# mrlooi/PoseCNN

Measured on AMD Instinct MI355X. Metric: frames/sec 640x480x21-class Hough-vote+RoI+ADD-loss, 1/2/4/8 MI355X, higher is better.
Workload: dtype f32 (FC GEMMs: exact 3-way split-bf16 x6 MFMA, products within 2^-24, fp32 accumulate: fp32-faithful)

## Files before the change

### include/posecnn_hip.h

```cpp
#ifndef POSECNN_HIP_H
#define POSECNN_HIP_H

#include <stddef.h>
#include <stdint.h>

#ifdef __cplusplus
extern "C" {
#endif

#define PCNN_OK 0
#define PCNN_EINVAL 1
#define PCNN_EHIP 2
#define PCNN_ECAPACITY 3

#define PCNN_MAX_ROI 128

int pcnn_abi_version(void);
const char* pcnn_strerror(int code);

int pcnn_set_completion_event(void* event);
int pcnn_completion_event_pending(void);

size_t pcnn_hough_voting_workspace_size(int B, int H, int W, int C, int skip_pixels, float vote_thr);

int pcnn_hough_voting(const int32_t* label, const float* vertex, const float* extents, const float* meta,
                      int num_meta, const float* gt, int num_gt, int B, int H, int W, int C, int batch_base,
                      int global_batch, int is_train, float inlier_thr, int label_thr, float vote_thr,
                      float per_thr, int skip_pixels, float* top_box, float* top_pose, float* top_target,
                      float* top_weight, int32_t* top_domain, int32_t* num_rois, int cap, int32_t* debug_counts,
                      void* workspace, size_t workspace_bytes, void* stream);

int pcnn_hough_voting_prob(const float* prob, int32_t* label_out, const float* vertex, const float* extents,
                           const float* meta, int num_meta, const float* gt, int num_gt, int B, int H, int W, int C,
                           int batch_base, int global_batch, int is_train, float inlier_thr, int label_thr,
                           float vote_thr, float per_thr, int skip_pixels, float* top_box, float* top_pose,
                           float* top_target, float* top_weight, int32_t* top_domain, int32_t* num_rois, int cap,
                           int32_t* debug_counts, void* workspace, size_t workspace_bytes, void* stream);

int pcnn_hough_voting_compact(const int32_t* label, const float* vertex3, const float* extents, const float* meta,
                              int num_meta, const float* gt, int num_gt, int B, int H, int W, int C, int batch_base,
                              int global_batch, int is_train, float inlier_thr, int label_thr, float vote_thr,
                              float per_thr, int skip_pixels, float* top_box, float* top_pose, float* top_target,
                              float* top_weight, int32_t* top_domain, int32_t* num_rois, int cap,
                              int32_t* debug_counts, void* workspace, size_t workspace_bytes, void* stream);

int pcnn_hough_voting_grad(float* grad_label, float* grad_vertex, int B, int H, int W, int C, void* stream);

int pcnn_hough_voting_diag(const void* workspace, int B, int H, int W, int C, int skip_pixels, float vote_thr,
                           int32_t* diag_host4, void* stream);

int pcnn_roi_pool_fwd(const float* data, int B, int H, int W, int C, int layout, const float* rois, int R_cap,
                      int roi_stride, int batch_base, const int32_t* num_rois_dev, float spatial_scale, int pooled_h, int pooled_w,
                      int pool_channel, float* top, int32_t* argmax, void* stream);

int pcnn_roi_pool_fwd_accumulate(const float* data, int B, int H, int W, int C, int layout, const float* rois,
                                 int R_cap, int roi_stride, int batch_base, const int32_t* num_rois_dev,
                                 float spatial_scale, int pooled_h, int pooled_w, int pool_channel, float* top,
                                 int32_t* argmax, void* stream);

int pcnn_roi_pool_fwd_pair(const float* data_a, int Ha, int Wa, float scale_a, const float* data_b, int Hb, int Wb,
                           float scale_b, int B, int C, const float* rois, int R_cap, int roi_stride,
                           int batch_base, const int32_t* num_rois_dev, int pooled_h, int pooled_w, float* top_sum,
                           int32_t* argmax_a, int32_t* argmax_b, void* stream);

int pcnn_roi_pool_fwd_pair_px(const float* data_a, int Ha, int Wa, float scale_a, const float* data_b, int Hb,
                              int Wb, float scale_b, int B, int C, const float* rois, int R_cap, int roi_stride,
                              int batch_base, const int32_t* num_rois_dev, int pooled_h, int pooled_w,
                              float* top_sum, uint16_t* argmax_a, uint16_t* argmax_b, void* stream);

size_t pcnn_roi_pool_bwd_workspace_size(int B, int R_cap);

int pcnn_roi_pool_bwd(const float* top_diff, const int32_t* argmax, int B, int H, int W, int C, int layout,
                      const float* rois, int R_cap, int roi_stride, int batch_base, const int32_t* num_rois_dev,
                      float spatial_scale, int pooled_h, int pooled_w, int pool_channel, float* bottom_diff,
                      void* workspace, size_t workspace_bytes, void* stream);

int pcnn_roi_pool_bwd_px(const float* top_diff, const uint16_t* argmax_px, int B, int H, int W, int C,
                         const float* rois, int R_cap, int roi_stride, int batch_base, const int32_t* num_rois_dev,
                         float spatial_scale, int pooled_h, int pooled_w, float* bottom_diff, void* workspace,
                         size_t workspace_bytes, void* stream);

size_t pcnn_add_loss_workspace_size(int R_cap, int C, int P);

int pcnn_add_loss_fwd(const float* pred, const float* target, const float* weight, const float* points,
                      const float* symmetry, int R_cap, const int32_t* num_rois_dev, int C, int P, float margin,
                      int loss_norm_rows, const int32_t* loss_norm_rows_dev, float* loss, float* bottom_diff,
                      void* workspace, size_t workspace_bytes, void* stream);

int pcnn_add_loss_prep(const float* weight, const float* symmetry, int R_cap, const int32_t* num_rois_dev, int C,
                       int P, void* workspace, size_t workspace_bytes, void* stream);
int pcnn_add_loss_fwd_prepared(const float* pred, const float* target, const float* weight, const float* points,
                               const float* symmetry, int R_cap, const int32_t* num_rois_dev, int C, int P,
                               float margin, int loss_norm_rows, const int32_t* loss_norm_rows_dev, float* loss,
                               float* bottom_diff, void* workspace, size_t workspace_bytes, void* stream);

int pcnn_add_loss_fwd_head_bwd(const float* pred, const float* target, const float* weight, const float* points,
                               const float* symmetry, int R_cap, const int32_t* num_rois_dev, int C, int P,
                               float margin, int loss_norm_rows, const int32_t* loss_norm_rows_dev,
                               float* bottom_diff, void* workspace, size_t workspace_bytes, const float* tanh_out,
                               const float* d_pred_scale, float* d_y8, void* stream);
int pcnn_add_loss_total(int R_cap, const int32_t* num_rois_dev, int C, int P, const void* workspace,
                        size_t workspace_bytes, float* loss, void* stream);

int pcnn_add_loss_bwd(const float* top_diff, const float* bottom_diff, int n, const int32_t* num_rois_dev,
                      int row_len, float* out, void* stream);

int pcnn_div_rn_check(const float* x, float b, int n, int dbl, float* out, void* stream);

int pcnn_backproject_fwd(const float* data, const float* label, const float* depth, const float* meta, int num_meta,
                         const float* label_3d, int B, int H, int W, int Ch, int NC, int grid_size,
                         int kernel_size, float threshold, float* top_data, float* top_label, float* top_flag,
                         void* stream);

int pcnn_backproject_bwd(const float* top_diff, const float* depth, const float* meta, int num_meta, int B, int H,
                         int W, int Ch, int grid_size, float* bottom_diff, void* stream);

size_t pcnn_gemm_workspace_size(int M, int N, int K, int m_dynamic, int precision);

int pcnn_gemm(int M, int N, int K, const float* A, const float* A2, int lda, int a_trans, const float* B, int ldb,
              int b_trans, float* Cm, int ldc, const float* bias, int act, const float* mask, int ldm,
              const int32_t* M_dev, const int32_t* K_dev, int precision, void* workspace, size_t workspace_bytes,
              void* stream);

int pcnn_gemm_drop(int M, int N, int K, const float* A, const float* A2, int lda, int a_trans, const float* B,
                   int ldb, int b_trans, float* Cm, int ldc, const float* bias, int act, const float* mask, int ldm,
                   const uint8_t* drop, int ldd, float keep_prob, const int32_t* M_dev, const int32_t* K_dev,
                   int precision, void* workspace, size_t workspace_bytes, void* stream);

int pcnn_gemm_drop_gen(int M, int N, int K, const float* A, const float* A2, int lda, int a_trans, const float* B,
                       int ldb, int b_trans, float* Cm, int ldc, const float* bias, int act, uint8_t* drop_out,
                       int ldd, float keep_prob, uint64_t seed, const int64_t* step_dev, int stream_id,
                       const int32_t* M_dev, const int32_t* K_dev, int precision, void* workspace,
                       size_t workspace_bytes, void* stream);

size_t pcnn_tp_bytes(int rows, int K);
int pcnn_split_tp(const float* src, long row_stride, long k_stride, int rows, const int32_t* rows_dev, int K,
                  const int32_t* K_dev, void* dst, size_t dst_bytes, void* stream);
int pcnn_gemm_tp(int M, int N, int K, const void* A_tp, const void* B_tp, float* Cm, int ldc, const float* bias,
                 int act, const float* mask, int ldm, const uint8_t* drop, int ldd, float keep_prob,
                 const int32_t* M_dev, const int32_t* K_dev, void* workspace, size_t workspace_bytes, void* stream);

int pcnn_dropout_mask(uint8_t* mask, int rows, int cols, int ld, const int32_t* rows_dev, uint64_t seed,
                      const int64_t* step_dev, int stream_id, float keep_prob, void* stream);

int pcnn_philox_check(const uint32_t* ctr, const uint32_t* key, int n, uint32_t* out, void* stream);

size_t pcnn_pose2d_workspace_size(int H, int W, int C, int n_hyp);
int pcnn_pose2d(const int32_t* label, const float* vertmap, const float* extents, int H, int W, int C, float fx,
                float fy, float px, float py, uint64_t seed, int n_hyp, int max_iter, float* poses_out,
                float* hyps_out, int32_t* hyp_px, int32_t* inl_out, int32_t* final_out, void* workspace,
                size_t workspace_bytes, void* stream);

size_t pcnn_pose3d_workspace_size(int H, int W, int C, int n_hyp);
int pcnn_pose3d(const int32_t* label, const uint16_t* depth, const float* vertmap, const float* extents, int H, int W,
                int C, float fx, float fy, float px, float py, float depth_factor, uint64_t seed, int n_hyp,
                int max_iter, int nm_evals, float* poses_out, float* hyps_out, int32_t* hyp_px, int32_t* inl_out,
                int32_t* final_out, float* energy_out, float* eye_out, void* workspace, size_t workspace_bytes,
                void* stream);

int pcnn_colsum(const float* X, int M, int N, int ldx, const int32_t* M_dev, float* out, void* stream);

int pcnn_pose_head_fwd(const float* y8, const float* poses_weight, int R_cap, const int32_t* num_rois_dev, int D,
                       float* tanh_out, float* pred, void* stream);

int pcnn_pose_head_bwd(const float* d_pred, const float* d_pred_scale, const float* tanh_out,
                       const float* poses_weight, const float* pred, int R_cap, const int32_t* num_rois_dev, int D,
                       float* d_y8, void* stream);

int pcnn_box_nms(const float* rois, int R_cap, int roi_stride, const int32_t* num_rois_dev, float thresh,
                 int32_t* keep, int32_t* num_keep, const float* poses_init, const float* poses_pred, int pred_dim,
                 float* rois_out, float* poses_out, void* stream);

int pcnn_argmax_2d(const float* prob, int B, int H, int W, int C, int32_t* label, void* stream);
int pcnn_hard_label_fwd(const float* prob, const int32_t* gt, int B, int H, int W, int C, float threshold,
                        float* top, void* stream);
int pcnn_hard_label_bwd(float* grad_prob, float* grad_gt, int B, int H, int W, int C, void* stream);

int pcnn_vertex_pred_compact(const float* feat, const float* weights, const float* bias, const int32_t* label, int B,
                             int H, int W, int K, int C, float* vertex3, void* stream);

int pcnn_icp_live_vertices(const uint16_t* depth, const int32_t* label, int H, int W, const int32_t* obj_ids, int L,
                           float factor, float fx, float fy, float px, float py, float* live, void* stream);
size_t pcnn_icp_workspace_size(int N, int H, int W);
int pcnn_icp(const float* live, int num_live, const int32_t* live_index, const float* pred_vertices,
             const float* pred_normals, int N, int H, int W, float fx, float fy, float px, float py, float znear, float zfar, float max_error,
             int iterations, const float* pose_in, float* update, float* pose_out, float* systems, void* workspace,
             size_t workspace_bytes, void* stream);
size_t pcnn_icp_reduce_workspace_size(int L, int H, int W);
int pcnn_icp_center(const float* live, const int32_t* label, const int32_t* obj_ids, int L, const float* vertmap,
                    const float* pred_vertices, const float* pred_normals, int H, int W, float max_error,
                    const float* pose_in, float* out, float* pose_out, void* workspace, size_t workspace_bytes,
                    void* stream);
size_t pcnn_energy_records_workspace_size(int N, int H, int W);
int pcnn_energy_records(const float* live, int n_live, const int32_t* label, const float* pred_vertices, int H, int W,
                        float znear, float zfar, int N, const int32_t* prob_obj, const int32_t* prob_live,
                        float* records, int32_t* counts, void* workspace, size_t workspace_bytes, void* stream);
int pcnn_energy_rec(const float* records, const int32_t* counts, int stride, const float* poses,
                    const int32_t* pose_prob, int K, float znear, float zfar, float* energy, void* stream);
int pcnn_nelder_mead_energy(const float* records, const int32_t* counts, int stride, int N, const double* x0,
                            const double* lb, const double* ub, int max_eval, float znear, float zfar, double* x_out,
                            double* f_out, int32_t* nev_out, void* stream);

size_t pcnn_nelder_mead_energy_workspace_size(int N);
int pcnn_nelder_mead_energy_coop(const float* records, const int32_t* counts, int stride, int N, const double* x0,
                                 const double* lb, const double* ub, int max_eval, float znear, float zfar,
                                 double* x_out, double* f_out, int32_t* nev_out, void* workspace,
                                 size_t workspace_bytes, void* stream);
int pcnn_nelder_mead_energy_coop_path(const float* records, const int32_t* counts, int stride, int N,
                                      const double* x0, const double* lb, const double* ub, int max_eval,
                                      float znear, float zfar, double* x_out, double* f_out, int32_t* nev_out,
                                      void* workspace, size_t workspace_bytes, int force_path, int32_t* path_out,
                                      void* stream);

size_t pcnn_icp_score_workspace_size(int J, int H, int W);
int pcnn_icp_score(const float* live, const int32_t* label, int obj, const float* vertmap, int H, int W,
                   const float* hyps, int J, float radius, float* score, int32_t* choose, void* workspace,
                   size_t workspace_bytes, void* stream);
int pcnn_pose_energy(const float* live, const int32_t* label, int obj, const float* pred_vertices, int H, int W,
                     float znear, float zfar, const float* poses, int K, float* energy, void* workspace,
                     size_t workspace_bytes, void* stream);

int pcnn_pose_energy_batch(const float* live, int n_live, const int32_t* label, const float* pred_vertices, int n_pv,
                           int H, int W, float znear, float zfar, const float* poses, int K, const int32_t* pose_obj,
                           const int32_t* pose_live, const int32_t* pose_pv, float* energy, void* workspace,
                           size_t workspace_bytes, void* stream);

size_t pcnn_render_workspace_size(int K, int H, int W, int V_total, int F_max);
int pcnn_render_meshes(const float* vertices, const float* normals, const int32_t* faces, const int32_t* vert_offset,
                       const int32_t* face_offset, int M, int V_total, int F_total, int F_max,
                       const int32_t* mesh_index, const int32_t* class_id, const float* poses, int K, int H, int W,
                       float fx, float fy, float px, float py, float znear, float zfar, float* pred_vertices,
                       float* pred_normals, float* vertmap, float* depth, int32_t* tri_id, void* workspace,
                       size_t workspace_bytes, void* stream);

#ifdef __cplusplus
}
#endif
#endif
```

### posecnn_amd/_lib.py

```python
import ctypes
import os
import threading

import torch

_HERE = os.path.dirname(os.path.abspath(__file__))
LIB_PATH = os.environ.get("POSECNN_HIP_LIB") or os.path.join(_HERE, "libposecnn_hip.so")

_lib = None
_lock = threading.Lock()

c_int = ctypes.c_int
c_float = ctypes.c_float
c_size_t = ctypes.c_size_t
c_void_p = ctypes.c_void_p

_SIGS = {
    "pcnn_abi_version": (c_int, []),
    "pcnn_strerror": (ctypes.c_char_p, [c_int]),
    "pcnn_set_completion_event": (c_int, [c_void_p]),
    "pcnn_completion_event_pending": (c_int, []),
    "pcnn_hough_voting_workspace_size": (c_size_t, [c_int, c_int, c_int, c_int, c_int, c_float]),
    "pcnn_hough_voting": (c_int, [c_void_p, c_void_p, c_void_p, c_void_p, c_int, c_void_p, c_int, c_int, c_int,
                                  c_int, c_int, c_int, c_int, c_int, c_float, c_int, c_float, c_float, c_int,
                                  c_void_p, c_void_p, c_void_p, c_void_p, c_void_p, c_void_p, c_int, c_void_p,
                                  c_void_p, c_size_t, c_void_p]),
    "pcnn_hough_voting_prob": (c_int, [c_void_p, c_void_p, c_void_p, c_void_p, c_void_p, c_int, c_void_p, c_int,
                                       c_int, c_int, c_int, c_int, c_int, c_int, c_int, c_float, c_int, c_float,
                                       c_float, c_int, c_void_p, c_void_p, c_void_p, c_void_p, c_void_p, c_void_p,
                                       c_int, c_void_p, c_void_p, c_size_t, c_void_p]),
    "pcnn_hough_voting_compact": (c_int, [c_void_p, c_void_p, c_void_p, c_void_p, c_int, c_void_p, c_int, c_int,
                                          c_int, c_int, c_int, c_int, c_int, c_int, c_float, c_int, c_float, c_float,
                                          c_int, c_void_p, c_void_p, c_void_p, c_void_p, c_void_p, c_void_p, c_int,
                                          c_void_p, c_void_p, c_size_t, c_void_p]),
    "pcnn_hough_voting_grad": (c_int, [c_void_p, c_void_p, c_int, c_int, c_int, c_int, c_void_p]),
    "pcnn_hough_voting_diag": (c_int, [c_void_p, c_int, c_int, c_int, c_int, c_int, c_float, c_void_p, c_void_p]),
    "pcnn_roi_pool_fwd": (c_int, [c_void_p, c_int, c_int, c_int, c_int, c_int, c_void_p, c_int, c_int, c_int,
                                  c_void_p, c_float, c_int, c_int, c_int, c_void_p, c_void_p, c_void_p]),
    "pcnn_roi_pool_fwd_accumulate": (c_int, [c_void_p, c_int, c_int, c_int, c_int, c_int, c_void_p, c_int, c_int,
                                             c_int, c_void_p, c_float, c_int, c_int, c_int, c_void_p, c_void_p, c_void_p]),
    "pcnn_roi_pool_fwd_pair": (c_int, [c_void_p, c_int, c_int, c_float, c_void_p, c_int, c_int, c_float, c_int, c_int,
                                       c_void_p, c_int, c_int, c_int, c_void_p, c_int, c_int, c_void_p, c_void_p,
                                       c_void_p, c_void_p]),
    "pcnn_roi_pool_fwd_pair_px": (c_int, [c_void_p, c_int, c_int, c_float, c_void_p, c_int, c_int, c_float, c_int,
                                          c_int, c_void_p, c_int, c_int, c_int, c_void_p, c_int, c_int, c_void_p,
                                          c_void_p, c_void_p, c_void_p]),
    "pcnn_roi_pool_bwd_workspace_size": (c_size_t, [c_int, c_int]),
    "pcnn_roi_pool_bwd_px": (c_int, [c_void_p, c_void_p, c_int, c_int, c_int, c_int, c_void_p, c_int, c_int, c_int,
                                     c_void_p, c_float, c_int, c_int, c_void_p, c_void_p, c_size_t, c_void_p]),
    "pcnn_roi_pool_bwd": (c_int, [c_void_p, c_void_p, c_int, c_int, c_int, c_int, c_int, c_void_p, c_int, c_int,
                                  c_int, c_void_p, c_float, c_int, c_int, c_int, c_void_p, c_void_p, c_size_t, c_void_p]),
    "pcnn_add_loss_workspace_size": (c_size_t, [c_int, c_int, c_int]),
    "pcnn_add_loss_fwd": (c_int, [c_void_p, c_void_p, c_void_p, c_void_p, c_void_p, c_int, c_void_p, c_int, c_int,
                                  c_float, c_int, c_void_p, c_void_p, c_void_p, c_void_p, c_size_t, c_void_p]),
    "pcnn_add_loss_fwd_prepared": (c_int, [c_void_p, c_void_p, c_void_p, c_void_p, c_void_p, c_int, c_void_p, c_int, c_int,
                                  c_float, c_int, c_void_p, c_void_p, c_void_p, c_void_p, c_size_t, c_void_p]),
    "pcnn_add_loss_prep": (c_int, [c_void_p, c_void_p, c_int, c_void_p, c_int, c_int, c_void_p, c_size_t, c_void_p]),
    "pcnn_add_loss_fwd_head_bwd": (c_int, [c_void_p, c_void_p, c_void_p, c_void_p, c_void_p, c_int, c_void_p, c_int,
                                           c_int, c_float, c_int, c_void_p, c_void_p, c_void_p, c_size_t, c_void_p,
                                           c_void_p, c_void_p, c_void_p]),
    "pcnn_add_loss_total": (c_int, [c_int, c_void_p, c_int, c_int, c_void_p, c_size_t, c_void_p, c_void_p]),
    "pcnn_add_loss_bwd": (c_int, [c_void_p, c_void_p, c_int, c_void_p, c_int, c_void_p, c_void_p]),
    "pcnn_div_rn_check": (c_int, [c_void_p, c_float, c_int, c_int, c_void_p, c_void_p]),
    "pcnn_backproject_fwd": (c_int, [c_void_p, c_void_p, c_void_p, c_void_p, c_int, c_void_p, c_int, c_int, c_int,
                                     c_int, c_int, c_int, c_int, c_float, c_void_p, c_void_p, c_void_p, c_void_p]),
    "pcnn_backproject_bwd": (c_int, [c_void_p, c_void_p, c_void_p, c_int, c_int, c_int, c_int, c_int, c_int,
                                     c_void_p, c_void_p]),
    "pcnn_gemm_workspace_size": (c_size_t, [c_int, c_int, c_int, c_int, c_int]),
    "pcnn_gemm": (c_int, [c_int, c_int, c_int, c_void_p, c_void_p, c_int, c_int, c_void_p, c_int, c_int, c_void_p,
                          c_int, c_void_p, c_int, c_void_p, c_int, c_void_p, c_void_p, c_int, c_void_p, c_size_t,
                          c_void_p]),
    "pcnn_gemm_drop": (c_int, [c_int, c_int, c_int, c_void_p, c_void_p, c_int, c_int, c_void_p, c_int, c_int,
                               c_void_p, c_int, c_void_p, c_int, c_void_p, c_int, c_void_p, c_int, c_float, c_void_p,
                               c_void_p, c_int, c_void_p, c_size_t, c_void_p]),
    "pcnn_gemm_drop_gen": (c_int, [c_int, c_int, c_int, c_void_p, c_void_p, c_int, c_int, c_void_p, c_int, c_int,
                                   c_void_p, c_int, c_void_p, c_int, c_void_p, c_int, c_float, ctypes.c_uint64,
                                   c_void_p, c_int, c_void_p, c_void_p, c_int, c_void_p, c_size_t, c_void_p]),
    "pcnn_dropout_mask": (c_int, [c_void_p, c_int, c_int, c_int, c_void_p, ctypes.c_uint64, c_void_p, c_int, c_float,
                                  c_void_p]),
    "pcnn_philox_check": (c_int, [c_void_p, c_void_p, c_int, c_void_p, c_void_p]),
    "pcnn_pose2d_workspace_size": (c_size_t, [c_int, c_int, c_int, c_int]),
    "pcnn_pose2d": (c_int, [c_void_p, c_void_p, c_void_p, c_int, c_int, c_int, c_float, c_float, c_float, c_float,
                            ctypes.c_uint64, c_int, c_int, c_void_p, c_void_p, c_void_p, c_void_p, c_void_p, c_void_p,
                            c_size_t, c_void_p]),
    "pcnn_pose3d_workspace_size": (c_size_t, [c_int, c_int, c_int, c_int]),
    "pcnn_pose3d": (c_int, [c_void_p, c_void_p, c_void_p, c_void_p, c_int, c_int, c_int, c_float, c_float, c_float,
                            c_float, c_float, ctypes.c_uint64, c_int, c_int, c_int, c_void_p, c_void_p, c_void_p,
                            c_void_p, c_void_p, c_void_p, c_void_p, c_void_p, c_size_t, c_void_p]),
    "pcnn_tp_bytes": (c_size_t, [c_int, c_int]),
    "pcnn_split_tp": (c_int, [c_void_p, ctypes.c_long, ctypes.c_long, c_int, c_void_p, c_int, c_void_p, c_void_p,
                              c_size_t, c_void_p]),
    "pcnn_gemm_tp": (c_int, [c_int, c_int, c_int, c_void_p, c_void_p, c_void_p, c_int, c_void_p, c_int, c_void_p,
                             c_int, c_void_p, c_int, c_float, c_void_p, c_void_p, c_void_p, c_size_t, c_void_p]),
    "pcnn_colsum": (c_int, [c_void_p, c_int, c_int, c_int, c_void_p, c_void_p, c_void_p]),
    "pcnn_box_nms": (c_int, [c_void_p, c_int, c_int, c_void_p, c_float, c_void_p, c_void_p, c_void_p, c_void_p, c_int,
                             c_void_p, c_void_p, c_void_p]),
    "pcnn_argmax_2d": (c_int, [c_void_p, c_int, c_int, c_int, c_int, c_void_p, c_void_p]),
    "pcnn_hard_label_fwd": (c_int, [c_void_p, c_void_p, c_int, c_int, c_int, c_int, c_float, c_void_p, c_void_p]),
    "pcnn_hard_label_bwd": (c_int, [c_void_p, c_void_p, c_int, c_int, c_int, c_int, c_void_p]),
    "pcnn_vertex_pred_compact": (c_int, [c_void_p, c_void_p, c_void_p, c_void_p, c_int, c_int, c_int, c_int, c_int,
                                         c_void_p, c_void_p]),
    "pcnn_pose_head_fwd": (c_int, [c_void_p, c_void_p, c_int, c_void_p, c_int, c_void_p, c_void_p, c_void_p]),
    "pcnn_pose_head_bwd": (c_int, [c_void_p, c_void_p, c_void_p, c_void_p, c_void_p, c_int, c_void_p, c_int, c_void_p,
                                   c_void_p]),
    "pcnn_icp_live_vertices": (c_int, [c_void_p, c_void_p, c_int, c_int, c_void_p, c_int, c_float, c_float, c_float,
                                       c_float, c_float, c_void_p, c_void_p]),
    "pcnn_icp_workspace_size": (c_size_t, [c_int, c_int, c_int]),
    "pcnn_icp": (c_int, [c_void_p, c_int, c_void_p, c_void_p, c_void_p, c_int, c_int, c_int, c_float, c_float, c_float,
                         c_float, c_float, c_float, c_float, c_int, c_void_p, c_void_p, c_void_p, c_void_p, c_void_p,
                         c_size_t, c_void_p]),
    "pcnn_icp_reduce_workspace_size": (c_size_t, [c_int, c_int, c_int]),
    "pcnn_icp_center": (c_int, [c_void_p, c_void_p, c_void_p, c_int, c_void_p, c_void_p, c_void_p, c_int, c_int,
                                c_float, c_void_p, c_void_p, c_void_p, c_void_p, c_size_t, c_void_p]),
    "pcnn_icp_score_workspace_size": (c_size_t, [c_int, c_int, c_int]),
    "pcnn_icp_score": (c_int, [c_void_p, c_void_p, c_int, c_void_p, c_int, c_int, c_void_p, c_int, c_float, c_void_p,
                               c_void_p, c_void_p, c_size_t, c_void_p]),
    "pcnn_energy_records_workspace_size": (c_size_t, [c_int, c_int, c_int]),
    "pcnn_energy_records": (c_int, [c_void_p, c_int, c_void_p, c_void_p, c_int, c_int, c_float, c_float, c_int,
                                    c_void_p, c_void_p, c_void_p, c_void_p, c_void_p, c_size_t, c_void_p]),
    "pcnn_energy_rec": (c_int, [c_void_p, c_void_p, c_int, c_void_p, c_void_p, c_int, c_float, c_float, c_void_p,
                                c_void_p]),
    "pcnn_nelder_mead_energy": (c_int, [c_void_p, c_void_p, c_int, c_int, c_void_p, c_void_p, c_void_p, c_int,
                                        c_float, c_float, c_void_p, c_void_p, c_void_p, c_void_p]),
    "pcnn_nelder_mead_energy_workspace_size": (c_size_t, [c_int]),
    "pcnn_nelder_mead_energy_coop": (c_int, [c_void_p, c_void_p, c_int, c_int, c_void_p, c_void_p, c_void_p, c_int,
                                             c_float, c_float, c_void_p, c_void_p, c_void_p, c_void_p, c_size_t,
                                             c_void_p]),
    "pcnn_nelder_mead_energy_coop_path": (c_int, [c_void_p, c_void_p, c_int, c_int, c_void_p, c_void_p, c_void_p,
                                                  c_int, c_float, c_float, c_void_p, c_void_p, c_void_p, c_void_p,
                                                  c_size_t, c_int, c_void_p, c_void_p]),
    "pcnn_pose_energy_batch": (c_int, [c_void_p, c_int, c_void_p, c_void_p, c_int, c_int, c_int, c_float, c_float,
                                       c_void_p, c_int, c_void_p, c_void_p, c_void_p, c_void_p, c_void_p, c_size_t,
                                       c_void_p]),
    "pcnn_pose_energy": (c_int, [c_void_p, c_void_p, c_int, c_void_p, c_int, c_int, c_float, c_float, c_void_p, c_int,
                                 c_void_p, c_void_p, c_size_t, c_void_p]),
    "pcnn_render_workspace_size": (c_size_t, [c_int, c_int, c_int, c_int, c_int]),
    "pcnn_render_meshes": (c_int, [c_void_p, c_void_p, c_void_p, c_void_p, c_void_p, c_int, c_int, c_int, c_int,
                                   c_void_p, c_void_p, c_void_p, c_int, c_int, c_int, c_float, c_float, c_float,
                                   c_float, c_float, c_float, c_void_p, c_void_p, c_void_p, c_void_p, c_void_p,
                                   c_void_p, c_size_t, c_void_p]),
}


class PcnnError(RuntimeError):
    pass


def load():
    global _lib
    if _lib is not None:
        return _lib
    with _lock:
        if _lib is None:
            if not os.path.exists(LIB_PATH):
                raise PcnnError(f"{LIB_PATH} not built; run __graft_entry__.build() "
                                "(hipcc --offload-arch=gfx950). No CPU fallback exists.")
            lib = ctypes.CDLL(LIB_PATH)
            for name, (res, args) in _SIGS.items():
                if name.endswith("_check") and not hasattr(lib, name):
                    continue
                fn = getattr(lib, name)
                fn.restype = res
                fn.argtypes = args
            _lib = lib
    return _lib


def exported_symbols():
    return list(_SIGS.keys())


def check(rc, what):
    if rc != 0:
        msg = load().pcnn_strerror(rc).decode()
        if rc == 1:
            raise ValueError(f"{what}: {msg}")
        raise PcnnError(f"{what}: {msg} (code {rc})")


def require_gpu(*tensors):
    if not torch.cuda.is_available():
        raise PcnnError("posecnn_amd ops run only on an AMD GPU (HIP); none is visible")
    for t in tensors:
        if t is not None and not t.is_cuda:
            raise ValueError("posecnn_amd ops take device tensors (got a CPU tensor)")


def ptr(t):
    return None if t is None else ctypes.c_void_p(t.data_ptr())


def stream_ptr(stream=None):
    s = stream if stream is not None else torch.cuda.current_stream()
    return ctypes.c_void_p(s.cuda_stream)


_ws = {}


def workspace(nbytes, device, tag="default", stream=None):
    s = stream if stream is not None else torch.cuda.current_stream(device)
    key = (str(device), tag, s.cuda_stream)
    buf = _ws.get(key)
    if buf is None or buf.numel() < nbytes:
        with torch.cuda.stream(s):
            buf = torch.empty(max(int(nbytes), 256), dtype=torch.uint8, device=device)
        _ws[key] = buf
    return buf
```

### posecnn_amd/csrc/roi_pooling.hip

```cpp
#include "pcnn_common.h"
#include <math.h>
#include <cfloat>

namespace {


struct RoiGeo {
  int b, cls, sw, sh, ew, eh;
  float bin_h, bin_w;
};

__device__ __forceinline__ RoiGeo roi_geo(const float* __restrict__ rois, int r, int stride, int batch_base,
                                          float scale, int PH, int PW) {
  const float* o = rois + (size_t)r * stride;
  RoiGeo g;
  g.b = (int)o[0] - batch_base;
  const int c0 = stride == 5 ? 1 : 2;
  g.cls = stride == 5 ? 0 : (int)o[1];
  g.sw = (int)roundf(o[c0 + 0] * scale);
  g.sh = (int)roundf(o[c0 + 1] * scale);
  g.ew = (int)roundf(o[c0 + 2] * scale);
  g.eh = (int)roundf(o[c0 + 3] * scale);
  const int roi_w = max(g.ew - g.sw + 1, 1);
  const int roi_h = max(g.eh - g.sh + 1, 1);
  g.bin_h = (float)roi_h / (float)PH;
  g.bin_w = (float)roi_w / (float)PW;
  return g;
}

__device__ __forceinline__ int rows_of(const int32_t* num_rois_dev, int R_cap) {
  if (!num_rois_dev) return R_cap;
  int r = *num_rois_dev;
  return r < R_cap ? r : R_cap;
}

__device__ __forceinline__ void bin_bounds(const RoiGeo& g, int ph, int pw, int H, int W, int& hs, int& he, int& ws,
                                           int& we) {
  hs = (int)floorf((float)ph * g.bin_h);
  ws = (int)floorf((float)pw * g.bin_w);
  he = (int)ceilf((float)(ph + 1) * g.bin_h);
  we = (int)ceilf((float)(pw + 1) * g.bin_w);
  hs = min(max(hs + g.sh, 0), H);
  he = min(max(he + g.sh, 0), H);
  ws = min(max(ws + g.sw, 0), W);
  we = min(max(we + g.sw, 0), W);
}

__device__ __forceinline__ void bins_of_pixel(const RoiGeo& g, int h, int w, int PH, int PW, int& phs, int& phe,
                                              int& pws, int& pwe) {
  phs = (int)floorf((float)(h - g.sh) / g.bin_h);
  phe = (int)ceilf((float)(h - g.sh + 1) / g.bin_h);
  pws = (int)floorf((float)(w - g.sw) / g.bin_w);
  pwe = (int)ceilf((float)(w - g.sw + 1) / g.bin_w);
  phs = min(max(phs, 0), PH);
  phe = min(max(phe, 0), PH);
  pws = min(max(pws, 0), PW);
  pwe = min(max(pwe, 0), PW);
}

__device__ __forceinline__ void upd(float v, int idx, float& m, int& a) {
  if (v > m) { m = v; a = idx; }
}

constexpr int kXcds = 8;
constexpr int kRun = 9;
__device__ __forceinline__ bool fwd_item(int R, int nbins, int& r, int& bin) {
  const int id = blockIdx.x;
  const int x = id % kXcds, local = id / kXcds;
  const int lr = local / nbins;
  bin = local % nbins;
  r = ((lr / kRun) * kXcds + x) * kRun + lr % kRun;
  return r < R;
}
static inline unsigned fwd_grid(int R_cap, int nbins) {
  return (unsigned)(kXcds * ((R_cap + kXcds * kRun - 1) / (kXcds * kRun)) * kRun * nbins);
}

template <bool PX = false>
__device__ __forceinline__ void bin_max4(const float* __restrict__ data, int B, int H, int W, int C,
                                         const RoiGeo& g, int ph, int pw, int c, float4& m, int4& a) {
  const bool bad = g.b < 0 || g.b >= B;
  int hs, he, ws, we;
  bin_bounds(g, ph, pw, H, W, hs, he, ws, we);
  const bool empty = bad || (he <= hs) || (we <= ws);
  const float* bd = data + (size_t)(bad ? 0 : g.b) * H * W * C;
  float m0, m1, m2, m3;
  m0 = m1 = m2 = m3 = empty ? 0.f : -FLT_MAX;
  int a0 = -1, a1 = -1, a2 = -1, a3 = -1;
  if (!empty) {
    for (int h = hs; h < he; h++) {
      int w = ws;
      for (; w + 1 < we; w += 2) {
        const int i0 = (h * W + w) * C + c, i1 = i0 + C;
        const float4 v0 = *(const float4*)(bd + i0);
        const float4 v1 = *(const float4*)(bd + i1);
        if (PX) {
          const int p0 = h * W + w, p1 = p0 + 1;
          upd(v0.x, p0, m0, a0); upd(v0.y, p0, m1, a1); upd(v0.z, p0, m2, a2); upd(v0.w, p0, m3, a3);
          upd(v1.x, p1, m0, a0); upd(v1.y, p1, m1, a1); upd(v1.z, p1, m2, a2); upd(v1.w, p1, m3, a3);
        } else {
          upd(v0.x, i0 + 0, m0, a0); upd(v0.y, i0 + 1, m1, a1); upd(v0.z, i0 + 2, m2, a2); upd(v0.w, i0 + 3, m3, a3);
          upd(v1.x, i1 + 0, m0, a0); upd(v1.y, i1 + 1, m1, a1); upd(v1.z, i1 + 2, m2, a2); upd(v1.w, i1 + 3, m3, a3);
        }
      }
      if (w < we) {
        const int i0 = (h * W + w) * C + c;
        const float4 v0 = *(const float4*)(bd + i0);
        if (PX) {
          const int p0 = h * W + w;
          upd(v0.x, p0, m0, a0); upd(v0.y, p0, m1, a1); upd(v0.z, p0, m2, a2); upd(v0.w, p0, m3, a3);
        } else {
          upd(v0.x, i0 + 0, m0, a0); upd(v0.y, i0 + 1, m1, a1); upd(v0.z, i0 + 2, m2, a2); upd(v0.w, i0 + 3, m3, a3);
        }
      }
    }
  }
  m = make_float4(m0, m1, m2, m3);
  a = make_int4(a0, a1, a2, a3);
}

template <bool ACC>
__global__ void __launch_bounds__(128) k_roi_fwd_nhwc4(const float* __restrict__ data, int B, int H, int W, int C,
                                                        const float* __restrict__ rois, int R_cap, int stride,
                                                        int batch_base, const int32_t* __restrict__ num_rois_dev,
                                                        float scale, int PH, int PW, float* __restrict__ top,
                                                        int32_t* __restrict__ argmax) {
  int r, bin;
  if (!fwd_item(rows_of(num_rois_dev, R_cap), PH * PW, r, bin)) return;
  const int ph = bin / PW, pw = bin % PW;
  const RoiGeo g = roi_geo(rois, r, stride, batch_base, scale, PH, PW);
  float* to = top + (((size_t)r * PH + ph) * PW + pw) * C;
  int32_t* ao = argmax + (((size_t)r * PH + ph) * PW + pw) * C;
  for (int c = threadIdx.x * 4; c < C; c += blockDim.x * 4) {
    float4 m;
    int4 a;
    bin_max4(data, B, H, W, C, g, ph, pw, c, m, a);
    if (ACC) {
      const float4 p = *(const float4*)(to + c);
      *(float4*)(to + c) = make_float4(p.x + m.x, p.y + m.y, p.z + m.z, p.w + m.w);
    } else {
      *(float4*)(to + c) = m;
    }
    *(int4*)(ao + c) = a;
  }
}

template <bool PX>
__global__ void __launch_bounds__(128) k_roi_fwd_pair_nhwc4(const float* __restrict__ data_a, int Ha, int Wa,
                                                             float scale_a, const float* __restrict__ data_b, int Hb,
                                                             int Wb, float scale_b, int B, int C,
                                                             const float* __restrict__ rois, int R_cap, int stride,
                                                             int batch_base, const int32_t* __restrict__ num_rois_dev,
                                                             int PH, int PW, float* __restrict__ top,
                                                             void* __restrict__ arg_a, void* __restrict__ arg_b) {
  int r, bin;
  if (!fwd_item(rows_of(num_rois_dev, R_cap), PH * PW, r, bin)) return;
  const int ph = bin / PW, pw = bin % PW;
  const RoiGeo ga = roi_geo(rois, r, stride, batch_base, scale_a, PH, PW);
  const RoiGeo gb = roi_geo(rois, r, stride, batch_base, scale_b, PH, PW);
  const size_t o = (((size_t)r * PH + ph) * PW + pw) * C;
  for (int c = threadIdx.x * 4; c < C; c += blockDim.x * 4) {
    float4 ma, mb;
    int4 aa, ab;
    bin_max4<PX>(data_a, B, Ha, Wa, C, ga, ph, pw, c, ma, aa);
    bin_max4<PX>(data_b, B, Hb, Wb, C, gb, ph, pw, c, mb, ab);
    *(float4*)(top + o + c) = make_float4(ma.x + mb.x, ma.y + mb.y, ma.z + mb.z, ma.w + mb.w);
    if (PX) {
      auto pk = [](int4 a) {
        return make_uint2(((unsigned)a.x & 0xFFFFu) | ((unsigned)a.y << 16),
                          ((unsigned)a.z & 0xFFFFu) | ((unsigned)a.w << 16));
      };
      *(uint2*)((uint16_t*)arg_a + o + c) = pk(aa);
      *(uint2*)((uint16_t*)arg_b + o + c) = pk(ab);
    } else {
      *(int4*)((int32_t*)arg_a + o + c) = aa;
      *(int4*)((int32_t*)arg_b + o + c) = ab;
    }
  }
}

__global__ void k_roi_fwd_generic(const float* __restrict__ data, int B, int H, int W, int C, int layout,
                                  const float* __restrict__ rois, int R_cap, int stride, int batch_base,
                                  const int32_t* __restrict__ num_rois_dev, float scale, int PH, int PW,
                                  int pool_channel, int acc, float* __restrict__ top, int32_t* __restrict__ argmax) {
  const int R = rows_of(num_rois_dev, R_cap);
  const int Co = pool_channel ? 1 : C;
  const long n_out = (long)R * PH * PW * Co;
  for (long idx = (long)blockIdx.x * blockDim.x + threadIdx.x; idx < n_out; idx += (long)gridDim.x * blockDim.x) {
    int r, ph, pw, c;
    if (layout == 0) {
      long t = idx;
      c = (int)(t % Co); t /= Co;
      pw = (int)(t % PW); t /= PW;
      ph = (int)(t % PH); r = (int)(t / PH);
    } else {
      long t = idx;
      pw = (int)(t % PW); t /= PW;
      ph = (int)(t % PH); t /= PH;
      c = (int)(t % Co); r = (int)(t / Co);
    }
    const RoiGeo g = roi_geo(rois, r, stride, batch_base, scale, PH, PW);
    const bool bad = g.b < 0 || g.b >= B;
    const int ch = pool_channel ? g.cls : c;
    int hs, he, ws, we;
    bin_bounds(g, ph, pw, H, W, hs, he, ws, we);
    const bool empty = bad || (he <= hs) || (we <= ws) || ch < 0 || ch >= C;
    float maxval = empty ? 0.f : -FLT_MAX;
    int maxidx = -1;
    if (!empty) {
      const float* bd = data + (size_t)g.b * H * W * C;
      for (int h = hs; h < he; h++)
        for (int w = ws; w < we; w++) {
          const int bi = layout == 0 ? (h * W + w) * C + ch : (ch * H + h) * W + w;
          const float v = bd[bi];
          if (v > maxval) { maxval = v; maxidx = bi; }
        }
    }
    top[idx] = acc ? top[idx] + maxval : maxval;
    argmax[idx] = maxidx;
  }
}

__global__ void __launch_bounds__(1024) k_roi_prep(const float* __restrict__ rois, int R_cap, int stride,
                                                    int batch_base, const int32_t* __restrict__ num_rois_dev, int B,
                                                    float scale, int PH, int PW, int32_t* __restrict__ geo,
                                                    int32_t* __restrict__ lo, int32_t* __restrict__ hi) {
  __shared__ int slo[1024], shi[1024];
  const int R = rows_of(num_rois_dev, R_cap);
  const int nb = B < 1024 ? B : 1024;
  for (int b = threadIdx.x; b < nb; b += blockDim.x) {
    slo[b] = 0x7fffffff;
    shi[b] = -1;
  }
  __syncthreads();
  for (int r = threadIdx.x; r < R; r += blockDim.x) {
    const RoiGeo g = roi_geo(rois, r, stride, batch_base, scale, PH, PW);
    int32_t* o = geo + (size_t)r * 8;
    o[0] = g.b; o[1] = g.cls; o[2] = g.sw; o[3] = g.sh; o[4] = g.ew; o[5] = g.eh;
    o[6] = __float_as_int(g.bin_h);
    o[7] = __float_as_int(g.bin_w);
    if (g.b >= 0 && g.b < nb) {
      atomicMin(&slo[g.b], r);
      atomicMax(&shi[g.b], r);
    }
  }
  __syncthreads();
  for (int b = threadIdx.x; b < B; b += blockDim.x) {
    lo[b] = b < nb ? slo[b] : 0;
    hi[b] = b < nb ? shi[b] : -1;
  }
}

#ifndef PCNN_RBW_NARROW
#define PCNN_RBW_NARROW 8192
#endif
constexpr int kBWaves = 1;
constexpr int kBChunk = 128 * kBWaves;
constexpr int kBGroup = 16;
constexpr int kBCap = kBGroup * 49;
constexpr int kBBatch = 8;

template <int kBTH, int kBTW, bool PX>
__global__ void __launch_bounds__(64 * kBWaves) k_roi_bwd_ent(const float* __restrict__ top_diff,
                                                               const void* __restrict__ argmax, int B, int H, int W,
                                                               int C, const int32_t* __restrict__ geo,
                                                               const int32_t* __restrict__ lo,
                                                               const int32_t* __restrict__ hi, int PH, int PW,
                                                               float* __restrict__ bottom) {
  constexpr int kBPix = kBTH * kBTW;
  __shared__ int2 ent[kBCap];
  __shared__ int sh_total;
  const int tiles_w = (W + kBTW - 1) / kBTW, tiles_h = (H + kBTH - 1) / kBTH;
  const int nchunk = (C + kBChunk - 1) / kBChunk;
  const int ipx = (int)((gridDim.x + 7) / 8);
  int id = (int)(blockIdx.x % 8) * ipx + (int)(blockIdx.x / 8);
  if (id >= B * tiles_w * tiles_h * nchunk) return;
  const int chunk = id % nchunk;
  id /= nchunk;
  const int t = id % (tiles_w * tiles_h), b = id / (tiles_w * tiles_h);
  const int h0 = (t / tiles_w) * kBTH, w0 = (t % tiles_w) * kBTW;
  const int th = min(kBTH, H - h0), tw = min(kBTW, W - w0);
  const int lane = pcnn::lane_id(), wave = threadIdx.x >> 6;
  const int c = chunk * kBChunk + 2 * threadIdx.x;
  const bool cok = c < C;
  float2 acc[kBPix];
  int expv[kBPix];
#pragma unroll
  for (int p = 0; p < kBPix; p++) {
    acc[p] = make_float2(0.f, 0.f);
    const int pix = (h0 + p / kBTW) * W + w0 + p % kBTW;
    expv[p] = PX ? pix : pix * C + c;
  }
  constexpr int kNext = PX ? 0 : 1;
  const int r0 = lo[b], r1 = hi[b];
  const __amdgpu_buffer_rsrc_t rs_t = __builtin_amdgcn_make_buffer_rsrc((void*)top_diff, (short)0, 0x7fffffff, 0x00020000);
  const __amdgpu_buffer_rsrc_t rs_a = __builtin_amdgcn_make_buffer_rsrc((void*)argmax, (short)0, 0x7fffffff, 0x00020000);
  const unsigned voff = cok ? (unsigned)c * 4u : 0x80000000u;
  const unsigned voff_a = cok ? (unsigned)c * (PX ? 2u : 4u) : 0x80000000u;
  for (int rb = r0; rb <= r1; rb += 64) {
    uint32_t rbits = 0;
    uint32_t cbits = 0;
    const int r = rb + lane;
    if (wave == 0 && r <= r1) {
      const int32_t* gg = geo + (size_t)r * 8;
      RoiGeo g;
      g.b = gg[0]; g.sw = gg[2]; g.sh = gg[3]; g.ew = gg[4]; g.eh = gg[5];
      g.bin_h = __int_as_float(gg[6]);
      g.bin_w = __int_as_float(gg[7]);
      if (g.b == b && g.sh <= h0 + th - 1 && g.eh >= h0 && g.sw <= w0 + tw - 1 && g.ew >= w0) {
        for (int i = 0; i < th; i++) {
          const int h = h0 + i;
          if (h < g.sh || h > g.eh) continue;
          int s0 = (int)floorf((float)(h - g.sh) / g.bin_h), e0 = (int)ceilf((float)(h - g.sh + 1) / g.bin_h);
          s0 = min(max(s0, 0), PH);
          e0 = min(max(e0, 0), PH);
          for (int ph = s0; ph < e0; ph++) rbits |= 1u << (ph * kBTH + i);
        }
        for (int j = 0; j < tw; j++) {
          const int w = w0 + j;
          if (w < g.sw || w > g.ew) continue;
          int s0 = (int)floorf((float)(w - g.sw) / g.bin_w), e0 = (int)ceilf((float)(w - g.sw + 1) / g.bin_w);
          s0 = min(max(s0, 0), PW);
          e0 = min(max(e0, 0), PW);
          for (int pw = s0; pw < e0; pw++) cbits |= 1u << (pw * kBTW + j);
        }
      }
    }
    const uint64_t hits = __ballot(rbits && cbits);
    for (int g0 = 0; g0 < 64; g0 += kBGroup) {
      if (wave == 0) {
        const uint64_t gm = hits & (((1ull << kBGroup) - 1) << g0);
        const bool mine = (gm >> lane) & 1;
        int cnt = 0;
        if (mine) {
          int nph = 0, npw = 0;
          for (int ph = 0; ph < PH; ph++) nph += ((rbits >> (ph * kBTH)) & ((1u << kBTH) - 1)) != 0;
          for (int pw = 0; pw < PW; pw++) npw += ((cbits >> (pw * kBTW)) & ((1u << kBTW) - 1)) != 0;
          cnt = nph * npw;
        }
        int off = cnt;
#pragma unroll
        for (int d = 1; d < 64; d <<= 1) {
          const int v = __shfl_up(off, d, 64);
          if (lane >= d) off += v;
        }
        if (lane == 63) sh_total = off;
        off -= cnt;
        if (mine) {
          const int rbase = r * PH;
          for (int ph = 0; ph < PH; ph++) {
            const uint32_t rm = (rbits >> (ph * kBTH)) & ((1u << kBTH) - 1);
            if (!rm) continue;
            for (int pw = 0; pw < PW; pw++) {
              const uint32_t cm = (cbits >> (pw * kBTW)) & ((1u << kBTW) - 1);
              if (!cm) continue;
              uint32_t m = 0;
#pragma unroll
              for (int i = 0; i < kBTH; i++)
                if ((rm >> i) & 1) m |= cm << (i * kBTW);
              ent[off++] = make_int2(((rbase + ph) * PW + pw) * C, (int)m);
            }
          }
        }
      }
      __syncthreads();
      const int total = sh_total;
      auto fetch = [&](int e0, int2& my, int2 (&av)[kBBatch], float2 (&dv)[kBBatch]) {
        my = ent[min(e0 + (lane & (kBBatch - 1)), total - 1)];
#pragma unroll
        for (int k = 0; k < kBBatch; k++) {
          const int so = __builtin_amdgcn_readlane(my.x, k) * 4;
          if (PX) {
            const unsigned a2 = __builtin_amdgcn_raw_buffer_load_b32(rs_a, voff_a, so >> 1, 0);
            av[k] = make_int2((int)(a2 & 0xFFFFu), (int)(a2 >> 16));
          } else {
            av[k] = __builtin_bit_cast(int2, __builtin_amdgcn_raw_buffer_load_b64(rs_a, voff_a, so, 0));
          }
          dv[k] = __builtin_bit_cast(float2, __builtin_amdgcn_raw_buffer_load_b64(rs_t, voff, so, 0));
        }
      };
      auto accumulate = [&](int e0, const int2& my, const int2 (&av)[kBBatch], const float2 (&dv)[kBBatch]) {
#pragma unroll
        for (int k = 0; k < kBBatch; k++) {
          if (e0 + k >= total) break;
          const uint32_t m = (uint32_t)__builtin_amdgcn_readlane(my.y, k);
#pragma unroll
          for (int q = 0; q < kBPix; q++) {
            if (!((m >> q) & 1)) continue;
            acc[q].x += av[k].x == expv[q] ? dv[k].x : 0.f;
            acc[q].y += av[k].y == expv[q] + kNext ? dv[k].y : 0.f;
          }
        }
      };
      if (total > 0) {
        int2 myA, myB, avA[kBBatch], avB[kBBatch];
        float2 dvA[kBBatch], dvB[kBBatch];
        fetch(0, myA, avA, dvA);
        for (int e0 = 0; e0 < total; e0 += 2 * kBBatch) {
          if (e0 + kBBatch < total) fetch(e0 + kBBatch, myB, avB, dvB);
          accumulate(e0, myA, avA, dvA);
          if (e0 + 2 * kBBatch < total) fetch(e0 + 2 * kBBatch, myA, avA, dvA);
          if (e0 + kBBatch < total) accumulate(e0 + kBBatch, myB, avB, dvB);
        }
      }
      __syncthreads();
    }
  }
  if (cok) {
#pragma unroll
    for (int i = 0; i < kBTH; i++)
#pragma unroll
      for (int j = 0; j < kBTW; j++)
        if (i < th && j < tw) *(float2*)(bottom + (((size_t)b * H + h0 + i) * W + w0 + j) * C + c) = acc[i * kBTW + j];
  }
}

__global__ void k_roi_bwd_generic(const float* __restrict__ top_diff, const int32_t* __restrict__ argmax, int B,
                                  int H, int W, int C, int layout, const int32_t* __restrict__ geo, int PH, int PW,
                                  int pool_channel, const int32_t* __restrict__ lo, const int32_t* __restrict__ hi,
                                  float* __restrict__ bottom) {
  const long npix = (long)B * H * W;
  const int Co = pool_channel ? 1 : C;
  for (long pi = (long)blockIdx.x * blockDim.x + threadIdx.x; pi < npix; pi += (long)gridDim.x * blockDim.x) {
    const int w = (int)(pi % W), h = (int)((pi / W) % H), b = (int)(pi / ((long)W * H));
    const int r0 = lo[b], r1 = hi[b];
    for (int r = r0; r <= r1; r++) {
      const int32_t* gg = geo + (size_t)r * 8;
      RoiGeo g;
      g.b = gg[0]; g.cls = gg[1]; g.sw = gg[2]; g.sh = gg[3]; g.ew = gg[4]; g.eh = gg[5];
      g.bin_h = __int_as_float(gg[6]);
      g.bin_w = __int_as_float(gg[7]);
      if (g.b != b) continue;
      if (!(w >= g.sw && w <= g.ew && h >= g.sh && h <= g.eh)) continue;
      int phs, phe, pws, pwe;
      bins_of_pixel(g, h, w, PH, PW, phs, phe, pws, pwe);
      const int cb = pool_channel ? g.cls : 0, ce = pool_channel ? g.cls + 1 : C;
      if (cb < 0 || ce > C) continue;
      for (int c = cb; c < ce; c++) {
        const int bidx = layout == 0 ? (h * W + w) * C + c : (c * H + h) * W + w;
        float* dst = bottom + (size_t)b * H * W * C + bidx;
        float acc = *dst;
        for (int ph = phs; ph < phe; ph++)
          for (int pw = pws; pw < pwe; pw++) {
            const int oc = pool_channel ? 0 : c;
            const size_t t = layout == 0 ? (((size_t)r * PH + ph) * PW + pw) * Co + oc
                                         : (((size_t)r * Co + oc) * PH + ph) * PW + pw;
            if (argmax[t] == bidx) acc += top_diff[t];
          }
        *dst = acc;
      }
    }
  }
}

}

static int roi_pool_fwd(const float* data, int B, int H, int W, int C, int layout, const float* rois, int R_cap,
                        int roi_stride, int batch_base, const int32_t* num_rois_dev, float spatial_scale,
                        int pooled_h, int pooled_w, int pool_channel, int acc, float* top, int32_t* argmax,
                        void* stream) {
  PCNN_REQUIRE(data && rois && top && argmax && B > 0 && H > 0 && W > 0 && C > 0 && R_cap >= 0);
  PCNN_REQUIRE(pooled_h > 0 && pooled_w > 0 && (layout == 0 || layout == 1));
  PCNN_REQUIRE(roi_stride >= 6 || (roi_stride == 5 && !pool_channel));
  PCNN_REQUIRE((long)H * W * C < (1l << 31));
  if (R_cap == 0) return PCNN_OK;
  hipStream_t st = (hipStream_t)stream;
  const bool vec = layout == 0 && !pool_channel && C % 4 == 0 && (((uintptr_t)data | (uintptr_t)top |
                                                                    (uintptr_t)argmax) & 15) == 0;
  if (vec) {
    const int threads = C / 4 >= 128 ? 128 : ((C / 4 + 63) / 64) * 64;
    if (acc)
      hipLaunchKernelGGL(k_roi_fwd_nhwc4<true>, dim3(fwd_grid(R_cap, pooled_h * pooled_w)), dim3(threads), 0, st, data, B, H,
                         W, C, rois, R_cap, roi_stride, batch_base, num_rois_dev, spatial_scale, pooled_h, pooled_w, top,
                         argmax);
    else
      hipLaunchKernelGGL(k_roi_fwd_nhwc4<false>, dim3(fwd_grid(R_cap, pooled_h * pooled_w)), dim3(threads), 0, st, data, B, H,
                         W, C, rois, R_cap, roi_stride, batch_base, num_rois_dev, spatial_scale, pooled_h, pooled_w, top,
                         argmax);
  } else {
    const long n = (long)R_cap * pooled_h * pooled_w * (pool_channel ? 1 : C);
    const int blocks = (int)((n + 255) / 256 < 8192 ? (n + 255) / 256 : 8192);
    hipLaunchKernelGGL(k_roi_fwd_generic, dim3(blocks), dim3(256), 0, st, data, B, H, W, C, layout, rois, R_cap,
                       roi_stride, batch_base, num_rois_dev, spatial_scale, pooled_h, pooled_w, pool_channel, acc, top,
                       argmax);
  }
  PCNN_CHECK_LAUNCH();
  return PCNN_OK;
}

extern "C" int pcnn_roi_pool_fwd(const float* data, int B, int H, int W, int C, int layout, const float* rois,
                                 int R_cap, int roi_stride, int batch_base, const int32_t* num_rois_dev,
                                 float spatial_scale, int pooled_h, int pooled_w, int pool_channel, float* top,
                                 int32_t* argmax, void* stream) {
  return roi_pool_fwd(data, B, H, W, C, layout, rois, R_cap, roi_stride, batch_base, num_rois_dev, spatial_scale,
                      pooled_h,
                      pooled_w, pool_channel, 0, top, argmax, stream);
}

extern "C" int pcnn_roi_pool_fwd_accumulate(const float* data, int B, int H, int W, int C, int layout,
                                            const float* rois, int R_cap, int roi_stride, int batch_base,
                                            const int32_t* num_rois_dev, float spatial_scale, int pooled_h,
                                            int pooled_w, int pool_channel, float* top, int32_t* argmax,
                                            void* stream) {
  return roi_pool_fwd(data, B, H, W, C, layout, rois, R_cap, roi_stride, batch_base, num_rois_dev, spatial_scale,
                      pooled_h,
                      pooled_w, pool_channel, 1, top, argmax, stream);
}

static int roi_pool_fwd_pair(const float* data_a, int Ha, int Wa, float scale_a, const float* data_b, int Hb, int Wb,
                             float scale_b, int B, int C, const float* rois, int R_cap, int roi_stride, int batch_base,
                             const int32_t* num_rois_dev, int pooled_h, int pooled_w, float* top_sum, void* argmax_a,
                             void* argmax_b, bool px, void* stream) {
  PCNN_REQUIRE(data_a && data_b && rois && top_sum && argmax_a && argmax_b && B > 0 && C > 0 && C % 4 == 0);
  PCNN_REQUIRE(Ha > 0 && Wa > 0 && Hb > 0 && Wb > 0 && pooled_h > 0 && pooled_w > 0 && R_cap >= 0);
  PCNN_REQUIRE(roi_stride >= 5);
  PCNN_REQUIRE((long)Ha * Wa * C < (1l << 31) && (long)Hb * Wb * C < (1l << 31));
  PCNN_REQUIRE(!px || ((long)Ha * Wa < 0xFFFF && (long)Hb * Wb < 0xFFFF));
  PCNN_REQUIRE(((((uintptr_t)data_a) | ((uintptr_t)data_b) | ((uintptr_t)top_sum)) & 15) == 0);
  PCNN_REQUIRE(((((uintptr_t)argmax_a) | ((uintptr_t)argmax_b)) & (px ? 7 : 15)) == 0);
  if (R_cap == 0) return PCNN_OK;
  const int threads = C / 4 >= 128 ? 128 : ((C / 4 + 63) / 64) * 64;
  if (px)
    hipLaunchKernelGGL(k_roi_fwd_pair_nhwc4<true>, dim3(fwd_grid(R_cap, pooled_h * pooled_w)), dim3(threads), 0,
                       (hipStream_t)stream, data_a, Ha, Wa, scale_a, data_b, Hb, Wb, scale_b, B, C, rois, R_cap,
                       roi_stride, batch_base, num_rois_dev, pooled_h, pooled_w, top_sum, argmax_a, argmax_b);
  else
    hipLaunchKernelGGL(k_roi_fwd_pair_nhwc4<false>, dim3(fwd_grid(R_cap, pooled_h * pooled_w)), dim3(threads), 0,
                       (hipStream_t)stream, data_a, Ha, Wa, scale_a, data_b, Hb, Wb, scale_b, B, C, rois, R_cap,
                       roi_stride, batch_base, num_rois_dev, pooled_h, pooled_w, top_sum, argmax_a, argmax_b);
  PCNN_CHECK_LAUNCH();
  return PCNN_OK;
}

extern "C" int pcnn_roi_pool_fwd_pair(const float* data_a, int Ha, int Wa, float scale_a, const float* data_b, int Hb,
                                      int Wb, float scale_b, int B, int C, const float* rois, int R_cap, int roi_stride,
                                      int batch_base, const int32_t* num_rois_dev, int pooled_h, int pooled_w, float* top_sum,
                                      int32_t* argmax_a, int32_t* argmax_b, void* stream) {
  return roi_pool_fwd_pair(data_a, Ha, Wa, scale_a, data_b, Hb, Wb, scale_b, B, C, rois, R_cap, roi_stride, batch_base,
                           num_rois_dev, pooled_h, pooled_w, top_sum, argmax_a, argmax_b, false, stream);
}

extern "C" int pcnn_roi_pool_fwd_pair_px(const float* data_a, int Ha, int Wa, float scale_a, const float* data_b,
                                         int Hb, int Wb, float scale_b, int B, int C, const float* rois, int R_cap,
                                         int roi_stride, int batch_base, const int32_t* num_rois_dev, int pooled_h,
                                         int pooled_w, float* top_sum, uint16_t* argmax_a, uint16_t* argmax_b,
                                         void* stream) {
  return roi_pool_fwd_pair(data_a, Ha, Wa, scale_a, data_b, Hb, Wb, scale_b, B, C, rois, R_cap, roi_stride, batch_base,
                           num_rois_dev, pooled_h, pooled_w, top_sum, argmax_a, argmax_b, true, stream);
}

extern "C" size_t pcnn_roi_pool_bwd_workspace_size(int B, int R_cap) {
  return pcnn::align_up((size_t)2 * (B > 0 ? B : 1) * sizeof(int32_t), 256) +
         pcnn::align_up((size_t)(R_cap > 0 ? R_cap : 1) * 8 * sizeof(int32_t), 256) + 256;
}

static int roi_pool_bwd(const float* top_diff, const void* argmax, bool px, int B, int H, int W, int C, int layout,
                        const float* rois, int R_cap, int roi_stride, int batch_base, const int32_t* num_rois_dev,
                        float spatial_scale, int pooled_h, int pooled_w, int pool_channel, float* bottom_diff,
                        void* workspace, size_t workspace_bytes, void* stream) {
  PCNN_REQUIRE(top_diff && argmax && rois && bottom_diff && workspace && B > 0 && H > 0 && W > 0 && C > 0);
  PCNN_REQUIRE(pooled_h > 0 && pooled_w > 0 && (layout == 0 || layout == 1) && R_cap >= 0);
  PCNN_REQUIRE(roi_stride >= 6 || (roi_stride == 5 && !pool_channel));
  PCNN_REQUIRE((long)H * W * C < (1l << 31));
  if (workspace_bytes < pcnn_roi_pool_bwd_workspace_size(B, R_cap)) return PCNN_ECAPACITY;
  hipStream_t st = (hipStream_t)stream;
  pcnn::Carve cv(workspace);
  int32_t* lo = cv.take<int32_t>(B);
  int32_t* hi = cv.take<int32_t>(B);
  int32_t* geo = cv.take<int32_t>((size_t)(R_cap > 0 ? R_cap : 1) * 8);
  hipLaunchKernelGGL(k_roi_prep, dim3(1), dim3(1024), 0, st, rois, R_cap, roi_stride, batch_base, num_rois_dev,
                     B, spatial_scale, pooled_h, pooled_w, geo, lo, hi);
  const int nchunk = (C + kBChunk - 1) / kBChunk;
  const long wg24 = (long)B * ((H + 1) / 2) * ((W + 3) / 4) * nchunk;
  const bool narrow = wg24 < PCNN_RBW_NARROW;
#ifndef PCNN_RBW_TH
#define PCNN_RBW_TH 2
#endif
  const int tbh = narrow ? 1 : PCNN_RBW_TH, tbw = 4;
  const bool vec = layout == 0 && !pool_channel && C % 2 == 0 && pooled_h * tbh <= 32 && pooled_w * tbw <= 32 &&
                   (long)H * W * C < (1l << 30) && (long)R_cap * pooled_h * pooled_w * C < (1l << 29) &&
                   (((uintptr_t)top_diff | (uintptr_t)bottom_diff) & 7) == 0 && ((uintptr_t)argmax & (px ? 3 : 7)) == 0;
  PCNN_REQUIRE(!px || (vec && (long)H * W < 0xFFFF));
  if (vec) {
    const int tiles = ((H + tbh - 1) / tbh) * ((W + tbw - 1) / tbw);
    const unsigned nwg = (unsigned)((B * tiles * nchunk + 7) / 8 * 8);
#define PCNN_RBW(TH, PXV)                                                                                  \
  pcnn::launch_last(k_roi_bwd_ent<TH, 4, PXV>, dim3(nwg), dim3(64 * kBWaves), 0, st, top_diff, argmax, B, H, W, C, \
                    geo, lo, hi, pooled_h, pooled_w, bottom_diff)
    if (narrow) {
      if (px) PCNN_RBW(1, true); else PCNN_RBW(1, false);
    } else {
      if (px) PCNN_RBW(PCNN_RBW_TH, true); else PCNN_RBW(PCNN_RBW_TH, false);
    }
#undef PCNN_RBW
  } else {
    if (hipMemsetAsync(bottom_diff, 0, (size_t)B * H * W * C * sizeof(float), st) != hipSuccess) return PCNN_EHIP;
    const long npix = (long)B * H * W;
    const int blocks = (int)((npix + 255) / 256 < 8192 ? (npix + 255) / 256 : 8192);
    hipLaunchKernelGGL(k_roi_bwd_generic, dim3(blocks), dim3(256), 0, st, top_diff, (const int32_t*)argmax, B, H, W,
                       C, layout, geo, pooled_h, pooled_w, pool_channel, lo, hi, bottom_diff);
  }
  PCNN_CHECK_LAUNCH();
  return PCNN_OK;
}

extern "C" int pcnn_roi_pool_bwd(const float* top_diff, const int32_t* argmax, int B, int H, int W, int C, int layout,
                                 const float* rois, int R_cap, int roi_stride, int batch_base,
                                 const int32_t* num_rois_dev, float spatial_scale, int pooled_h, int pooled_w,
                                 int pool_channel, float* bottom_diff, void* workspace, size_t workspace_bytes, void* stream) {
  return roi_pool_bwd(top_diff, argmax, false, B, H, W, C, layout, rois, R_cap, roi_stride, batch_base, num_rois_dev,
                      spatial_scale, pooled_h, pooled_w, pool_channel, bottom_diff, workspace, workspace_bytes, stream);
}

extern "C" int pcnn_roi_pool_bwd_px(const float* top_diff, const uint16_t* argmax_px, int B, int H, int W, int C,
                                    const float* rois, int R_cap, int roi_stride, int batch_base,
                                    const int32_t* num_rois_dev, float spatial_scale, int pooled_h, int pooled_w,
                                    float* bottom_diff, void* workspace, size_t workspace_bytes, void* stream) {
  return roi_pool_bwd(top_diff, argmax_px, true, B, H, W, C, 0, rois, R_cap, roi_stride, batch_base, num_rois_dev,
                      spatial_scale, pooled_h, pooled_w, 0, bottom_diff, workspace, workspace_bytes, stream);
}
```

### posecnn_amd/pipeline.py

```python
import contextlib

import torch

from . import _lib
from . import pose_head as ph
from .hough_voting_gpu_layer import hough_voting_gpu_op as hv
from .roi_pooling_layer import roi_pooling_op as rp
from .average_distance_loss import average_distance_loss_op as adl
from .exchange import GradShard, RoiExchange

CAP = hv.CAPACITY
_nullctx = contextlib.nullcontext


class PoseStep:
    def __init__(self, B, H, W, num_classes, device, conv4_hw=None, conv5_hw=None, channels=512, units=4096,
                 is_train=1, skip_pixels=10, vote_threshold=-1.0, vote_percentage=0.02, margin=0.01,
                 global_batch=None, batch_base=0, weights=None, dist=None, backward=True, precision=2,
                 overlap_weight_grads=True, pixel_argmax=True, keep_prob=None, drop_seed=0x5EED, side_prep=True,
                 drop_in_reduce=True, pipeline=False, prefetch_at="loss", fuse_loss_tail=True,
                 defer_side_join=False, signal_forks=True, pool_at_tail=False):
        self.B, self.H, self.W, self.C = B, H, W, num_classes
        self.dev = device
        self.is_train, self.skip, self.vthr, self.vper, self.margin = is_train, skip_pixels, vote_threshold, \
            vote_percentage, margin
        self.global_batch = global_batch or B
        self.batch_base = batch_base
        self.dist = dist
        self.backward = backward
        self.prec = precision
        self.h4, self.w4 = conv4_hw or (H // 8, W // 8)
        self.h5, self.w5 = conv5_hw or (H // 16, W // 16)
        self.Ch = channels
        D = 4 * num_classes
        self.D = D
        self.weights = weights or ph.PoseHeadWeights(num_classes, device, in_dim=49 * channels, units=units)
        f32 = dict(dtype=torch.float32, device=device)
        i32 = dict(dtype=torch.int32, device=device)
        K6 = 49 * channels
        px = pixel_argmax and max(self.h4 * self.w4, self.h5 * self.w5) < 0xFFFF
        adt = dict(dtype=torch.int16 if px else torch.int32, device=device)

        def minibatch_set():
            return dict(hough=dict(box=torch.zeros((CAP, 7), **f32), pose=torch.zeros((CAP, 7), **f32),
                                   target=torch.zeros((CAP, D), **f32), weight=torch.zeros((CAP, D), **f32),
                                   domain=torch.zeros((CAP,), **i32), num_rois=torch.zeros((2,), **i32)),
                        pool=torch.zeros((CAP, 7, 7, channels), **f32),
                        arg5=torch.zeros((CAP, 7, 7, channels), **adt),
                        arg4=torch.zeros((CAP, 7, 7, channels), **adt),
                        add_ws=None, prepped=False)
        self.fuse_loss_tail = fuse_loss_tail
        self.pipeline = bool(pipeline)
        self._sets = [minibatch_set() for _ in range(2 if self.pipeline else 1)]
        self._cur = 0
        self._primed = None
        self.prefetch_at = prefetch_at
        if prefetch_at not in ("loss", "bwd", "start", "fwd", "tail"):
            raise ValueError("prefetch_at must be 'start', 'fwd', 'loss', 'bwd' or 'tail'")
        self._fork_ev = torch.cuda.Event() if self.pipeline else None
        self._fork_recorded = False
        self.pre_stream = torch.cuda.Stream(device=device) if self.pipeline else None
        self._next = None
        self.y6 = torch.zeros((CAP, units), **f32)
        self.y7 = torch.zeros((CAP, units), **f32)
        self.y8 = torch.zeros((CAP, D), **f32)
        self.t8 = torch.zeros((CAP, D), **f32)
        self.pred = torch.zeros((CAP, D), **f32)
        self.loss = torch.zeros((1,), **f32)
        self.diff = torch.zeros((CAP, D), **f32)
        self.one = torch.ones((1,), **f32)
        self.dy8 = torch.zeros((CAP, D), **f32)
        self.dy7 = torch.zeros((CAP, units), **f32)
        self.dy6 = torch.zeros((CAP, units), **f32)
        self.dx = torch.zeros((CAP, K6), **f32)
        self.gshard = None
        if dist is not None:
            per_max = 9 if is_train else 1
            slot = max(1, min(CAP, B * (hv.MAX_ROI // self.global_batch) * per_max))
            self.gshard = GradShard(dist, slot, [("w6", (K6, units)), ("w7", (units, units)), ("w8", (units, D))],
                                    device)
        self.grads = self.weights.grads_like()
        if self.gshard is not None:
            for k in ("w6", "w7", "w8"):
                self.grads[k] = self.grads[k][self.gshard.rows(k)].contiguous()
        self.keep = float(keep_prob if keep_prob is not None else (0.5 if is_train else 1.0))
        if not 0.0 < self.keep <= 1.0:
            raise ValueError("keep_prob must be in (0, 1]")
        self.drop6 = self.drop7 = None
        self._drop_external = False
        self.drop_in_reduce = drop_in_reduce
        self._bump_drop_step = False
        self._drawn = False
        if self.keep < 1.0:
            u8 = dict(dtype=torch.uint8, device=device)
            self.drop6 = torch.zeros((CAP, units), **u8)
            self.drop7 = torch.zeros((CAP, units), **u8)
            self.drop_step = torch.zeros((1,), dtype=torch.int64, device=device)
            rank = dist.get_rank() if dist is not None else 0
            self.drop_seed = (int(drop_seed) + rank * 0x9E3779B97F4A7C15) & ((1 << 64) - 1)
            self._drop_ready = None
            self._drop_ev = torch.cuda.Event()
        self.dconv4 = torch.zeros((B, self.h4, self.w4, channels), **f32)
        self.dconv5 = torch.zeros((B, self.h5, self.w5, channels), **f32)
        self.norm_rows = torch.zeros((1,), **i32)
        self.timer = None
        self.gemm_timer = None
        self.xchg = None
        self.detections = None
        self._pending = {}
        self._in_step = False
        self.side_stream = torch.cuda.Stream(device=device) if overlap_weight_grads else None
        self.side_prep = side_prep and self.side_stream is not None
        self.defer_side_join = bool(defer_side_join) and self.pipeline and dist is None and \
            self.side_stream is not None
        self._side_mid_ev = torch.cuda.Event() if self.defer_side_join else None
        self._side_done_ev = torch.cuda.Event() if self.defer_side_join else None
        self._side_pending = False
        self.signal_forks = bool(signal_forks) and self.side_stream is not None and dist is None
        self._fork_evs = {}
        self.pool_at_tail = bool(pool_at_tail) and self.pipeline
        self._pool_pending = None
        if self.signal_forks:
            for k in ("loss", "fc8_dx", "fc7_dx"):
                ev = torch.cuda.Event()
                ev.record()
                self._fork_evs[k] = ev
        self._mid_covers_pre = False
        self._mid_waited = False

    def _t(self, name):
        step = self

        class _Ctx:
            def __enter__(self_):
                if step.timer is not None:
                    self_.e0 = torch.cuda.Event(enable_timing=True)
                    self_.e0.record()

            def __exit__(self_, *a):
                if step.timer is not None:
                    e1 = torch.cuda.Event(enable_timing=True)
                    e1.record()
                    step.timer.setdefault(name, []).append((self_.e0, e1))
        return _Ctx()

    def join(self):
        cur = torch.cuda.current_stream()
        for st in (self.side_stream, self.pre_stream):
            if st is not None:
                cur.wait_stream(st)
        self._side_pending = False

    def _side_wait(self, ev_name, stream=None):
        if self._side_pending:
            (stream or torch.cuda.current_stream()).wait_event(getattr(self, ev_name))

    def _arm_fork(self, name):
        if not self.signal_forks or self.timer is not None or torch.cuda.is_current_stream_capturing():
            return None
        ev = self._fork_evs[name]
        _lib.load().pcnn_set_completion_event(ev.cuda_event)
        return ev

    @staticmethod
    def _fork_taken(ev):
        if ev is None:
            return None
        return None if _lib.load().pcnn_completion_event_pending() else ev

    def _fork_side(self, side, ev):
        if ev is not None:
            side.wait_event(ev)
        else:
            side.wait_stream(torch.cuda.current_stream())

    hough = property(lambda self: self._sets[self._cur]["hough"])
    pool = property(lambda self: self._sets[self._cur]["pool"])
    arg5 = property(lambda self: self._sets[self._cur]["arg5"])
    arg4 = property(lambda self: self._sets[self._cur]["arg4"])
    add_ws = property(lambda self: self._sets[self._cur]["add_ws"])

    def vote(self, label, vertex, extents, meta, gt, s=None):
        s = self._cur if s is None else s
        self._sets[s]["pooled"] = False
        with self._t("hough_voting_gpu"):
            return hv.hough_voting_gpu_capacity(label, vertex, extents, meta, gt, self.is_train, self.vthr,
                                                self.vper, self.skip, global_batch=self.global_batch,
                                                batch_base=self.batch_base, out=self._sets[s]["hough"])

    def add_prep(self, points, symmetry, s=None, stream=None):
        s = self._cur if s is None else s
        st = self._sets[s]
        if st["add_ws"] is None:
            st["add_ws"] = torch.empty(adl.workspace_bytes(CAP, self.C, points.shape[1]), dtype=torch.uint8,
                                       device=self.dev)
        h = st["hough"]
        side = None
        if stream is None:
            side = self.side_stream if self.timer is None and self.side_prep else None
            if side is not None:
                side.wait_stream(torch.cuda.current_stream())
        with torch.cuda.stream(stream or side or torch.cuda.current_stream()):
            adl.average_distance_loss_prep(h["weight"], symmetry, points.shape[1], st["add_ws"],
                                           num_rois=h["num_rois"][1:2])
        st["prepped"] = "side" if side is not None else "stream"

    def pool_fwd(self, conv4, conv5, s=None):
        s = self._cur if s is None else s
        st = self._sets[s]
        with self._t("roi_pool_fwd"):
            rp.roi_pool_pair(conv5, 1.0 / 16.0, conv4, 1.0 / 8.0, st["hough"]["box"], 7, 7,
                             num_rois=st["hough"]["num_rois"][1:2], out=(st["pool"], st["arg5"], st["arg4"]),
                             batch_base=self.batch_base)
        st["pooled"] = True

    def _front(self, inputs, s, stream=None):
        ctx = torch.cuda.stream(stream) if stream is not None else _nullctx()
        with ctx:
            self.vote(inputs["label"], inputs["vertex"], inputs["extents"], inputs["meta"], inputs["gt"], s=s)
            if stream is not None:
                self.add_prep(inputs["points"], inputs["symmetry"], s=s, stream=stream)
                if self.pool_at_tail and stream is self.pre_stream:
                    self._pool_pending = (inputs, s)
                else:
                    self.pool_fwd(inputs["conv4"], inputs["conv5"], s=s)

    def _issue_pending_pool(self):
        if self._pool_pending is None:
            return
        inputs, s = self._pool_pending
        self._pool_pending = None
        with torch.cuda.stream(self.pre_stream):
            self.pool_fwd(inputs["conv4"], inputs["conv5"], s=s)

    def _prefetch(self):
        if self._next is None:
            return
        nxt, s = self._next
        self._next = None
        if self.timer is not None:
            self._side_wait("_side_done_ev")
            self._side_pending = False
            self._front(nxt, s, stream=torch.cuda.current_stream())
        else:
            if self._fork_recorded:
                self.pre_stream.wait_event(self._fork_ev)
            else:
                self.pre_stream.wait_stream(torch.cuda.current_stream())
            self._side_wait("_side_done_ev", self.pre_stream)
            self._front(nxt, s, stream=self.pre_stream)
        self._fork_recorded = False
        self._primed = (s, nxt)

    def set_drop_masks(self, m6, m7):
        if self.keep >= 1.0:
            raise ValueError("set_drop_masks: the step has keep_prob 1 (no dropout)")
        for dst, m in ((self.drop6, m6), (self.drop7, m7)):
            dst.zero_()
            dst[:m.shape[0]].copy_(m.to(torch.uint8))
        self._drop_external = True

    def draw_drop_masks(self):
        if self.keep >= 1.0 or self._drop_external or self.drop_in_reduce:
            return
        self._drawn = True
        nr = self.hough["num_rois"][1:2]
        side = self.side_stream if self.timer is None and self.side_prep else None
        if side is not None:
            side.wait_stream(torch.cuda.current_stream())
        with torch.cuda.stream(side or torch.cuda.current_stream()):
            ph.dropout_mask(self.drop6, self.keep, self.drop_seed, self.drop_step, 6, rows_dev=nr)
            ph.dropout_mask(self.drop7, self.keep, self.drop_seed, self.drop_step, 7, rows_dev=nr)
            self.drop_step.add_(1)
            if side is not None:
                self._drop_ev.record(side)
                self._drop_ready = self._drop_ev

    def exchange(self):
        h = self.hough
        if self.dist is None:
            self.norm_rows = h["num_rois"][1:2]
            return
        with self._t("allreduce_rows"):
            self.norm_rows.copy_(h["num_rois"][0:1])
            self._pending["rows"] = self.dist.all_reduce(self.norm_rows, async_op=True)

    def _wait(self, key):
        w = self._pending.pop(key, None)
        if w is not None:
            w.wait()

    def gather_detections(self):
        h = self.hough
        if self.dist is None:
            return torch.cat([h["box"], h["pose"]], 1), h["num_rois"][0:1]
        return self._exchange_rows()(h["box"], h["pose"], h["num_rois"])

    def _exchange_rows(self):
        if self.xchg is None:
            self.xchg = RoiExchange(self.dist, CAP, self.dev)
        return self.xchg

    def forward(self, conv4, conv5, points, symmetry):
        h = self.hough
        nr = h["num_rois"][1:2]
        w = self.weights
        K6 = 49 * self.Ch
        st = self._sets[self._cur]
        if not (self.pipeline and st.get("pooled")):
            self.pool_fwd(conv4, conv5)
        x = self.pool.view(CAP, K6)
        gs = self.gshard if self.backward else None
        if gs is not None:
            gs.send_input("w6", x)
        dk = dict(keep_prob=self.keep) if self.keep < 1.0 else {}
        if not self._drawn:
            self.draw_drop_masks()
        self._drawn = False
        if self.keep < 1.0 and getattr(self, "_drop_ready", None) is not None:
            torch.cuda.current_stream().wait_event(self._drop_ready)
            self._drop_ready = None
        gen = self.keep < 1.0 and self.drop_in_reduce and not self._drop_external
        g6 = dict(drop_gen=(self.drop_seed, self.drop_step, 6)) if gen else {}
        g7 = dict(drop_gen=(self.drop_seed, self.drop_step, 7)) if gen else {}
        if not self._mid_waited:
            self._side_wait("_side_mid_ev")
        self._mid_waited = False
        with self._t("gemm_fc6_fwd"):
            self._g("fc6_fwd", x, w.w6, self.y6, bias=w.b6, act=1, M_dev=nr, drop=self.drop6, **dk, **g6)
        if self.prefetch_at == "fwd":
            self._prefetch()
        if gs is not None:
            gs.send_input("w7", self.y6)
        with self._t("gemm_fc7_fc8_fwd"):
            self._g("fc7_fwd", self.y6, w.w7, self.y7, bias=w.b7, act=1, M_dev=nr, drop=self.drop7, **dk, **g7)
            if gs is not None:
                gs.send_input("w8", self.y7)
            self._g("fc8_fwd", self.y7, w.w8, self.y8, bias=w.b8, act=0, M_dev=nr)
        if self.prefetch_at == "loss":
            self._prefetch()
        if gen:
            if self._in_step and self.backward:
                self._bump_drop_step = True
            else:
                self.drop_step.add_(1)
        if self.dist is not None:
            self._wait("rows")
            self.norm_rows.clamp_(min=1)
        with self._t("head_add_loss_fwd"):
            ph.head_fwd(self.y8, h["weight"], self.t8, self.pred, num_rois=nr)
            if not st["prepped"]:
                self.add_prep(points, symmetry)
            if st["prepped"] == "side":
                torch.cuda.current_stream().wait_stream(self.side_stream)
            st["prepped"] = False
            self._wait("loss")
            side = self.side_stream
            self._head_bwd_done = fuse = (self.fuse_loss_tail and self._in_step and self.backward and
                                          self.timer is None and side is not None and self.D <= 256)
            if fuse:
                ev = self._arm_fork("loss")
                adl.average_distance_loss_head_bwd(self.pred, h["target"], h["weight"], points, symmetry,
                                                   self.margin, self.t8, self.one, self.diff, self.dy8, st["add_ws"],
                                                   num_rois=nr, loss_norm_rows_dev=self.norm_rows)
                self._fork_side(side, self._fork_taken(ev))
                with torch.cuda.stream(side):
                    adl.average_distance_loss_total(CAP, self.C, points.shape[1], st["add_ws"], self.loss,
                                                    num_rois=nr)
                    if self.dist is not None:
                        self._pending["loss"] = self.dist.all_reduce(self.loss, async_op=True)
                return self.loss
            adl.average_distance_loss(self.pred, h["target"], h["weight"], points, symmetry, self.margin,
                                      num_rois=nr, loss_norm_rows_dev=self.norm_rows, out=(self.loss, self.diff),
                                      workspace=st["add_ws"], prepared=True)
        if self.dist is not None:
            self._pending["loss"] = self.dist.all_reduce(self.loss, async_op=True)
            if not self._in_step:
                self._wait("loss")
        return self.loss

    def backward_pass(self, conv4, conv5):
        h = self.hough
        nr = h["num_rois"][1:2]
        w, g = self.weights, self.grads
        K6 = 49 * self.Ch
        main = torch.cuda.current_stream()
        side = self.side_stream if self.timer is None else None
        gs = self.gshard
        x = self.pool.view(CAP, K6)

        def weight_grads(name, X, dY, K_loc, M, N, fork=True, fork_ev=None):
            if side is not None and fork:
                self._fork_side(side, fork_ev)
            if gs is not None:
                gs.send_grad(name, dY, nr)
            with torch.cuda.stream(side or main):
                if gs is not None:
                    gs.reduce(name, g[name], g["b" + name[1:]],
                              lambda A, B_, C_, **kw: self._g(f"fc{name[1:]}_dw", A, B_, C_, **kw), ph.colsum)
                else:
                    ph.colsum(dY, g["b" + name[1:]], M_dev=nr)
                    self._g(f"fc{name[1:]}_dw", X, dY, g[name], a_trans=1, K_dev=nr, M=M, N=N, K=K_loc)

        fused_fork = getattr(self, "_head_bwd_done", False) and side is not None
        if not getattr(self, "_head_bwd_done", False):
            with self._t("add_loss_head_bwd"):
                ph.head_bwd(self.diff, self.t8, h["weight"], self.pred, self.dy8, num_rois=nr,
                            d_pred_scale=self.one)
        self._head_bwd_done = False
        if self.prefetch_at == "bwd":
            self._prefetch()
        with self._t("gemm_fc8_fc7_dw_bias"):
            weight_grads("w8", self.y7, self.dy8, CAP, w.units, self.D, fork=not fused_fork)
        dk = dict(keep_prob=self.keep) if self.keep < 1.0 else {}
        ev = self._arm_fork("fc8_dx") if side is not None else None
        with self._t("gemm_fc8_fc7_dx"):
            self._g("fc8_dx", self.dy8, w.w8, self.dy7, b_trans=1, mask=self.y7, M_dev=nr, **dk)
        ev = self._fork_taken(ev)
        with self._t("gemm_fc8_fc7_dw_bias"):
            weight_grads("w7", self.y6, self.dy7, CAP, w.units, w.units, fork_ev=ev)
        defer = self.defer_side_join and side is not None
        self._side_wait("_side_done_ev")
        self._side_pending = False
        if defer:
            self._mid_covers_pre = (self._primed is not None and self._pool_pending is None and
                                    not torch.cuda.is_current_stream_capturing())
            if self._mid_covers_pre:
                side.wait_stream(self.pre_stream)
            if self._bump_drop_step and self._mid_covers_pre:
                with torch.cuda.stream(side):
                    self.drop_step.add_(1)
                self._bump_drop_step = False
            self._side_mid_ev.record(side)
        ev = self._arm_fork("fc7_dx") if side is not None else None
        with self._t("gemm_fc8_fc7_dx"):
            self._g("fc7_dx", self.dy7, w.w7, self.dy6, b_trans=1, mask=self.y6, M_dev=nr, **dk)
        ev = self._fork_taken(ev)
        with self._t("gemm_fc6_dw"):
            weight_grads("w6", x, self.dy6, CAP, K6, w.units, fork_ev=ev)
        with self._t("gemm_fc6_dx"):
            self._g("fc6_dx", self.dy6, w.w6, self.dx, b_trans=1, M_dev=nr)
        if self.prefetch_at == "tail":
            self._prefetch()
        self._issue_pending_pool()
        dxp = self.dx.view(CAP, 7, 7, self.Ch)
        with self._t("roi_pool_bwd"):
            rp.roi_pool_grad(conv5, h["box"], self.arg5, dxp, 7, 7, 1.0 / 16.0, 0, num_rois=nr, out=self.dconv5,
                             batch_base=self.batch_base)
            rp.roi_pool_grad(conv4, h["box"], self.arg4, dxp, 7, 7, 1.0 / 8.0, 0, num_rois=nr, out=self.dconv4,
                             batch_base=self.batch_base)
        if self._bump_drop_step:
            self.drop_step.add_(1)
            self._bump_drop_step = False
        if defer:
            self._side_done_ev.record(side)
            self._side_pending = True
        elif side is not None:
            main.wait_stream(side)

    def _g(self, name, A, B, C, **kw):
        if self.gemm_timer is None:
            return ph.gemm(A, B, C, precision=self.prec, **kw)
        e0, e1 = torch.cuda.Event(enable_timing=True), torch.cuda.Event(enable_timing=True)
        e0.record()
        ph.gemm(A, B, C, precision=self.prec, **kw)
        e1.record()
        self.gemm_timer.setdefault(name, []).append((e0, e1))
        return C

    def step(self, inputs, next_inputs=None):
        if self.pipeline:
            return self._step_pipelined(inputs, next_inputs)
        if next_inputs is not None:
            raise ValueError("next_inputs needs PoseStep(pipeline=True)")
        self.vote(inputs["label"], inputs["vertex"], inputs["extents"], inputs["meta"], inputs["gt"])
        self.draw_drop_masks()
        if self.side_prep:
            self.add_prep(inputs["points"], inputs["symmetry"])
        return self._train(inputs)

    def _step_pipelined(self, inputs, next_inputs):
        main = torch.cuda.current_stream()
        if self._primed is not None and self._primed[1] is inputs:
            self._cur = self._primed[0]
            if self._side_pending and self._mid_covers_pre:
                main.wait_event(self._side_mid_ev)
                self._mid_waited = True
            else:
                main.wait_stream(self.pre_stream)
        else:
            self._side_wait("_side_done_ev")
            self._side_pending = False
            self._front(inputs, self._cur, stream=main)
        self._primed = None
        self._next = (next_inputs, 1 - self._cur) if next_inputs is not None else None
        self.draw_drop_masks()
        if self.prefetch_at == "start":
            self._prefetch()
        elif self.prefetch_at == "fwd" and self._next is not None and self.timer is None:
            self._fork_ev.record(main)
            self._fork_recorded = True
        loss = self._train(inputs)
        self._prefetch()
        self._issue_pending_pool()
        return loss

    def _train(self, inputs):
        self.exchange()
        if self.dist is not None:
            with self._t("allgather_rois"):
                h = self.hough
                self._exchange_rows().start(h["box"], h["pose"], h["num_rois"])
        self._in_step = True
        try:
            loss = self.forward(inputs["conv4"], inputs["conv5"], inputs["points"], inputs["symmetry"])
            if self.backward:
                self.backward_pass(inputs["conv4"], inputs["conv5"])
        finally:
            self._in_step = False
        self._wait("loss")
        if self.dist is not None:
            rows, total = self.xchg.finish()
            self.detections = (rows.clone(), total.clone())
        return loss
```

### posecnn_amd/roi_pooling_layer/roi_pooling_op.py

```python
import torch

from .. import _lib


def roi_pool(bottom_data, bottom_rois, pooled_height, pooled_width, spatial_scale, pool_channel=0, name=None,
             num_rois=None, layout=0, out=None, accumulate=False, batch_base=0):
    _lib.require_gpu(bottom_data, bottom_rois)
    if bottom_data.dim() != 4:
        raise ValueError("data must be 4-dimensional")
    if bottom_rois.dim() != 2:
        raise ValueError("rois must be 2-dimensional")
    data = bottom_data.contiguous().float()
    rois = bottom_rois.contiguous().float()
    if layout == 0:
        B, H, W, C = data.shape
    else:
        B, C, H, W = data.shape
    R, stride = rois.shape
    Co = 1 if pool_channel else C
    shape = (R, pooled_height, pooled_width, Co) if layout == 0 else (R, Co, pooled_height, pooled_width)
    if out is None:
        if accumulate:
            raise ValueError("accumulate=True needs out=(top, argmax)")
        top = torch.empty(shape, dtype=torch.float32, device=data.device)
        arg = torch.empty(shape, dtype=torch.int32, device=data.device)
    else:
        top, arg = out
    lib = _lib.load()
    fn = lib.pcnn_roi_pool_fwd_accumulate if accumulate else lib.pcnn_roi_pool_fwd
    rc = fn(_lib.ptr(data), B, H, W, C, layout, _lib.ptr(rois), R, stride, int(batch_base), _lib.ptr(num_rois),
            float(spatial_scale), int(pooled_height), int(pooled_width), int(pool_channel), _lib.ptr(top),
            _lib.ptr(arg), _lib.stream_ptr())
    _lib.check(rc, "roi_pool")
    return top, arg


def roi_pool_pair(data_a, scale_a, data_b, scale_b, rois, pooled_height, pooled_width, num_rois=None, out=None,
                  batch_base=0, pixel_argmax=False):
    _lib.require_gpu(data_a, data_b, rois)
    if data_a.dim() != 4 or data_b.dim() != 4 or rois.dim() != 2:
        raise ValueError("data must be 4-dimensional and rois 2-dimensional")
    da, db = data_a.contiguous().float(), data_b.contiguous().float()
    B, Ha, Wa, C = da.shape
    Bb, Hb, Wb, Cb = db.shape
    if (Bb, Cb) != (B, C):
        raise ValueError("both maps need the same batch and channel count")
    rois = rois.contiguous().float()
    R, stride = rois.shape
    shape = (R, pooled_height, pooled_width, C)
    if out is None:
        adt = torch.int16 if pixel_argmax else torch.int32
        out = (torch.empty(shape, dtype=torch.float32, device=da.device),
               torch.empty(shape, dtype=adt, device=da.device),
               torch.empty(shape, dtype=adt, device=da.device))
    top, arg_a, arg_b = out
    if arg_a.dtype != arg_b.dtype or arg_a.dtype not in (torch.int16, torch.int32):
        raise ValueError("argmax tensors must both be int32 (flat index) or int16 (pixel index)")
    fn = _lib.load().pcnn_roi_pool_fwd_pair_px if arg_a.dtype == torch.int16 else _lib.load().pcnn_roi_pool_fwd_pair
    rc = fn(_lib.ptr(da), Ha, Wa, float(scale_a), _lib.ptr(db), Hb, Wb, float(scale_b), B, C, _lib.ptr(rois), R, stride,
            int(batch_base), _lib.ptr(num_rois), int(pooled_height), int(pooled_width), _lib.ptr(top), _lib.ptr(arg_a),
            _lib.ptr(arg_b), _lib.stream_ptr())
    _lib.check(rc, "roi_pool_pair")
    return top, arg_a, arg_b


def roi_pool_grad(bottom_data, bottom_rois, argmax, grad, pooled_height, pooled_width, spatial_scale,
                  pool_channel=0, name=None, num_rois=None, layout=0, out=None, batch_base=0):
    _lib.require_gpu(bottom_data, bottom_rois, argmax, grad)
    rois = bottom_rois.contiguous().float()
    if layout == 0:
        B, H, W, C = bottom_data.shape
    else:
        B, C, H, W = bottom_data.shape
    R, stride = rois.shape
    lib = _lib.load()
    ws = _lib.workspace(lib.pcnn_roi_pool_bwd_workspace_size(B, R), bottom_data.device, "roi_bwd")
    dd = out if out is not None else torch.empty(bottom_data.shape, dtype=torch.float32, device=bottom_data.device)
    if argmax.dtype == torch.int16:
        if layout != 0 or pool_channel:
            raise ValueError("a pixel-index argmax needs NHWC data and pool_channel 0")
        rc = lib.pcnn_roi_pool_bwd_px(_lib.ptr(grad.contiguous()), _lib.ptr(argmax.contiguous()), B, H, W, C,
                                      _lib.ptr(rois), R, stride, int(batch_base), _lib.ptr(num_rois),
                                      float(spatial_scale), int(pooled_height), int(pooled_width), _lib.ptr(dd),
                                      _lib.ptr(ws), ws.numel(), _lib.stream_ptr())
    else:
        rc = lib.pcnn_roi_pool_bwd(_lib.ptr(grad.contiguous()), _lib.ptr(argmax.contiguous()), B, H, W, C, layout,
                                   _lib.ptr(rois), R, stride, int(batch_base), _lib.ptr(num_rois),
                                   float(spatial_scale), int(pooled_height), int(pooled_width), int(pool_channel),
                                   _lib.ptr(dd), _lib.ptr(ws), ws.numel(), _lib.stream_ptr())
    _lib.check(rc, "roi_pool_grad")
    return dd


class RoiPoolFunction(torch.autograd.Function):

    @staticmethod
    def forward(ctx, data, rois, pooled_height, pooled_width, spatial_scale, pool_channel=0, layout=0):
        top, arg = roi_pool(data, rois, pooled_height, pooled_width, spatial_scale, pool_channel, layout=layout)
        ctx.save_for_backward(data, rois, arg)
        ctx.params = (pooled_height, pooled_width, spatial_scale, pool_channel, layout)
        return top, arg

    @staticmethod
    def backward(ctx, grad, _garg):
        data, rois, arg = ctx.saved_tensors
        ph, pw, sc, pc, layout = ctx.params
        return roi_pool_grad(data, rois, arg, grad, ph, pw, sc, pc, layout=layout), None, None, None, None, None, None
```

Before: 4630.

## Precompute per-tile RoI-bin entry lists for RoI-pool backward, optionally on side stream

Adds a planning pass that turns the RoI geometry into per-row and per-column bin bitmasks, then builds a compact per-tile list of (bin, pixel-mask) entries with an atomic cursor and wave prefix sums. The backward kernel then walks only the tile's entry list instead of scanning every RoI and recomputing bin bounds inside each block. It also changes the channel width per lane. The pipeline runs the planning right after the forward pool, or on a side stream during prep, so it can overlap other work. The cost is extra plan buffers, an extra launch, and more complex synchronisation through an event.

```diff
diff --git a/include/posecnn_hip.h b/include/posecnn_hip.h
--- a/include/posecnn_hip.h
+++ b/include/posecnn_hip.h
@@ -79,6 +79,23 @@
                          const float* rois, int R_cap, int roi_stride, int batch_base, const int32_t* num_rois_dev,
                          float spatial_scale, int pooled_h, int pooled_w, float* bottom_diff, void* workspace,
                          size_t workspace_bytes, void* stream);
+
+size_t pcnn_roi_pool_bwd_plan_size(int B, int H, int W, int C, int R_cap, int pooled_h, int pooled_w, int tile_h);
+
+size_t pcnn_roi_pool_bwd_plan_entry_cap(int B, int H, int W, int C, int R_cap, int pooled_h, int pooled_w,
+                                        int tile_h);
+
+int pcnn_roi_pool_bwd_plan(const float* rois, int R_cap, int roi_stride, int batch_base, const int32_t* num_rois_dev,
+                           int B, int H, int W, int C, float spatial_scale, int pooled_h, int pooled_w, int tile_h,
+                           void* plan, size_t plan_bytes, void* stream);
+
+int pcnn_roi_pool_bwd_planned(const float* top_diff, const int32_t* argmax, int B, int H, int W, int C, int R_cap,
+                              int pooled_h, int pooled_w, int tile_h, int lane_channels, const void* plan,
+                              size_t plan_bytes, float* bottom_diff, void* stream);
+
+int pcnn_roi_pool_bwd_planned_px(const float* top_diff, const uint16_t* argmax_px, int B, int H, int W, int C,
+                                 int R_cap, int pooled_h, int pooled_w, int tile_h, int lane_channels,
+                                 const void* plan, size_t plan_bytes, float* bottom_diff, void* stream);
 
 size_t pcnn_add_loss_workspace_size(int R_cap, int C, int P);
 
diff --git a/posecnn_amd/_lib.py b/posecnn_amd/_lib.py
--- a/posecnn_amd/_lib.py
+++ b/posecnn_amd/_lib.py
@@ -50,6 +50,14 @@
                                      c_void_p, c_float, c_int, c_int, c_void_p, c_void_p, c_size_t, c_void_p]),
     "pcnn_roi_pool_bwd": (c_int, [c_void_p, c_void_p, c_int, c_int, c_int, c_int, c_int, c_void_p, c_int, c_int,
                                   c_int, c_void_p, c_float, c_int, c_int, c_int, c_void_p, c_void_p, c_size_t, c_void_p]),
+    "pcnn_roi_pool_bwd_plan_size": (c_size_t, [c_int, c_int, c_int, c_int, c_int, c_int, c_int, c_int]),
+    "pcnn_roi_pool_bwd_plan_entry_cap": (c_size_t, [c_int, c_int, c_int, c_int, c_int, c_int, c_int, c_int]),
+    "pcnn_roi_pool_bwd_plan": (c_int, [c_void_p, c_int, c_int, c_int, c_void_p, c_int, c_int, c_int, c_int, c_float,
+                                       c_int, c_int, c_int, c_void_p, c_size_t, c_void_p]),
+    "pcnn_roi_pool_bwd_planned": (c_int, [c_void_p, c_void_p, c_int, c_int, c_int, c_int, c_int, c_int, c_int, c_int,
+                                          c_int, c_void_p, c_size_t, c_void_p, c_void_p]),
+    "pcnn_roi_pool_bwd_planned_px": (c_int, [c_void_p, c_void_p, c_int, c_int, c_int, c_int, c_int, c_int, c_int,
+                                             c_int, c_int, c_void_p, c_size_t, c_void_p, c_void_p]),
     "pcnn_add_loss_workspace_size": (c_size_t, [c_int, c_int, c_int]),
     "pcnn_add_loss_fwd": (c_int, [c_void_p, c_void_p, c_void_p, c_void_p, c_void_p, c_int, c_void_p, c_int, c_int,
                                   c_float, c_int, c_void_p, c_void_p, c_void_p, c_void_p, c_size_t, c_void_p]),
diff --git a/posecnn_amd/csrc/roi_plan.h b/posecnn_amd/csrc/roi_plan.h
--- /dev/null
+++ b/posecnn_amd/csrc/roi_plan.h
@@ -0,0 +1,87 @@
+#pragma once
+#include <math.h>
+#include <stddef.h>
+#include <stdint.h>
+
+#if defined(__HIPCC__)
+#define ROI_PLAN_HD __host__ __device__
+#else
+#define ROI_PLAN_HD
+#endif
+
+namespace roi_plan {
+
+constexpr int kTileW = 4;
+constexpr int kMaxPooled = 8;
+constexpr int kWideChunk = 256;
+constexpr long kFedFrom = 16384;
+
+inline long wide_groups(int B, int H, int W, int C, int th) {
+  return (long)B * ((H + th - 1) / th) * ((W + kTileW - 1) / kTileW) * ((C + kWideChunk - 1) / kWideChunk);
+}
+
+inline int tile_h(int B, int H, int W, int C, int req) {
+  if (req == 1 || req == 2) return req;
+  return wide_groups(B, H, W, C, 2) >= kFedFrom ? 2 : 1;
+}
+
+inline bool wide_by_size(int B, int H, int W, int C, int th) { return wide_groups(B, H, W, C, th) >= kFedFrom; }
+
+inline bool plannable(int B, int H, int W, int C, int R_cap, int PH, int PW) {
+  return B > 0 && H > 0 && W > 0 && C > 0 && C % 2 == 0 && R_cap >= 0 && PH > 0 && PW > 0 && PH <= kMaxPooled &&
+         PW <= kMaxPooled && (long)H * W * C < (1l << 30) && (long)R_cap * PH * PW * C < (1l << 29) &&
+         (long)R_cap * PH * PW < (1l << 24) && (long)B * H * W < (1l << 28);
+}
+
+inline long tiles_of(int H, int W, int th) { return (long)((H + th - 1) / th) * ((W + kTileW - 1) / kTileW); }
+
+inline size_t entries_per_roi(int H, int W, int PH, int PW, int th) {
+  const size_t tiles_h = (size_t)((H + th - 1) / th), tiles_w = (size_t)((W + kTileW - 1) / kTileW);
+  return ((size_t)PH + tiles_h) * ((size_t)PW + tiles_w);
+}
+
+inline size_t entry_cap(int H, int W, int R_cap, int PH, int PW, int th) {
+  return (size_t)(R_cap > 0 ? R_cap : 1) * entries_per_roi(H, W, PH, PW, th);
+}
+
+inline size_t align_up(size_t x, size_t a) { return (x + a - 1) / a * a; }
+
+struct Layout {
+  size_t cursor, lo, hi, geo, rowbits, colbits, first, count, ent, ent_cap, bytes;
+};
+
+inline Layout layout(int B, int H, int W, int R_cap, int PH, int PW, int th) {
+  const size_t R = (size_t)(R_cap > 0 ? R_cap : 1), nb = (size_t)(B > 0 ? B : 1);
+  const size_t nt = nb * (size_t)tiles_of(H, W, th);
+  Layout L;
+  size_t off = 0;
+  auto take = [&off](size_t bytes) {
+    const size_t at = off;
+    off = align_up(off + bytes, 256);
+    return at;
+  };
+  L.cursor = take(2 * sizeof(int32_t));
+  L.lo = take(nb * sizeof(int32_t));
+  L.hi = take(nb * sizeof(int32_t));
+  L.geo = take(R * 8 * sizeof(int32_t));
+  L.rowbits = take(R * (size_t)H);
+  L.colbits = take(R * (size_t)W);
+  L.first = take(nt * sizeof(int32_t));
+  L.count = take(nt * sizeof(int32_t));
+  L.ent_cap = entry_cap(H, W, R_cap, PH, PW, th);
+  L.ent = take(L.ent_cap * sizeof(uint32_t));
+  L.bytes = off;
+  return L;
+}
+
+ROI_PLAN_HD inline uint32_t accept_bits(int p, int start, int end, float bin, int P) {
+  if (p < start || p > end) return 0u;
+  int s0 = (int)floorf((float)(p - start) / bin), e0 = (int)ceilf((float)(p - start + 1) / bin);
+  s0 = s0 < 0 ? 0 : (s0 > P ? P : s0);
+  e0 = e0 < 0 ? 0 : (e0 > P ? P : e0);
+  return e0 > s0 ? ((1u << e0) - 1u) & ~((1u << s0) - 1u) : 0u;
+}
+
+ROI_PLAN_HD inline uint32_t pack_entry(uint32_t bin, uint32_t mask) { return (bin << 8) | mask; }
+
+}
diff --git a/posecnn_amd/csrc/roi_pooling.hip b/posecnn_amd/csrc/roi_pooling.hip
--- a/posecnn_amd/csrc/roi_pooling.hip
+++ b/posecnn_amd/csrc/roi_pooling.hip
@@ -1,4 +1,5 @@
 #include "pcnn_common.h"
+#include "roi_plan.h"
 #include <math.h>
 #include <cfloat>
 
@@ -224,8 +225,10 @@
 __global__ void __launch_bounds__(1024) k_roi_prep(const float* __restrict__ rois, int R_cap, int stride,
                                                     int batch_base, const int32_t* __restrict__ num_rois_dev, int B,
                                                     float scale, int PH, int PW, int32_t* __restrict__ geo,
-                                                    int32_t* __restrict__ lo, int32_t* __restrict__ hi) {
+                                                    int32_t* __restrict__ lo, int32_t* __restrict__ hi,
+                                                    int32_t* __restrict__ cursor) {
   __shared__ int slo[1024], shi[1024];
+  if (cursor && threadIdx.x == 0) *cursor = 0;
   const int R = rows_of(num_rois_dev, R_cap);
   const int nb = B < 1024 ? B : 1024;
   for (int b = threadIdx.x; b < nb; b += blockDim.x) {
@@ -251,27 +254,125 @@
   }
 }
 
-#ifndef PCNN_RBW_NARROW
-#define PCNN_RBW_NARROW 8192
-#endif
-constexpr int kBWaves = 1;
-constexpr int kBChunk = 128 * kBWaves;
-constexpr int kBGroup = 16;
-constexpr int kBCap = kBGroup * 49;
-constexpr int kBBatch = 8;
-
-template <int kBTH, int kBTW, bool PX>
-__global__ void __launch_bounds__(64 * kBWaves) k_roi_bwd_ent(const float* __restrict__ top_diff,
-                                                               const void* __restrict__ argmax, int B, int H, int W,
-                                                               int C, const int32_t* __restrict__ geo,
-                                                               const int32_t* __restrict__ lo,
-                                                               const int32_t* __restrict__ hi, int PH, int PW,
-                                                               float* __restrict__ bottom) {
+
+__global__ void __launch_bounds__(128) k_roi_plan_bits(const int32_t* __restrict__ geo, int R_cap,
+                                                        const int32_t* __restrict__ num_rois_dev, int H, int W,
+                                                        int PH, int PW, uint8_t* __restrict__ rowbits,
+                                                        uint8_t* __restrict__ colbits) {
+  const int r = blockIdx.x;
+  if (r >= rows_of(num_rois_dev, R_cap)) return;
+  const int32_t* gg = geo + (size_t)r * 8;
+  const int sw = gg[2], sh = gg[3], ew = gg[4], eh = gg[5];
+  const float bin_h = __int_as_float(gg[6]), bin_w = __int_as_float(gg[7]);
+  for (int t = threadIdx.x; t < H + W; t += blockDim.x) {
+    if (t < H)
+      rowbits[(size_t)r * H + t] = (uint8_t)roi_plan::accept_bits(t, sh, eh, bin_h, PH);
+    else
+      colbits[(size_t)r * W + t - H] = (uint8_t)roi_plan::accept_bits(t - H, sw, ew, bin_w, PW);
+  }
+}
+
+constexpr int kPlanWaves = 16;
+template <int kBTH>
+__global__ void __launch_bounds__(64 * kPlanWaves) k_roi_plan_list(
+    const int32_t* __restrict__ geo, const int32_t* __restrict__ lo, const int32_t* __restrict__ hi,
+    const uint8_t* __restrict__ rowbits, const uint8_t* __restrict__ colbits, int B, int H, int W, int PH, int PW,
+    int32_t* __restrict__ cursor, int32_t* __restrict__ first, int32_t* __restrict__ count,
+    uint32_t* __restrict__ ent, int ent_cap) {
+  constexpr int kBTW = roi_plan::kTileW;
+  const int tiles_w = (W + kBTW - 1) / kBTW, tiles_h = (H + kBTH - 1) / kBTH;
+  __shared__ int s_total[kPlanWaves], s_base;
+  const int wave = (int)(threadIdx.x >> 6);
+  const int item = blockIdx.x * kPlanWaves + wave;
+  const bool live = item < B * tiles_w * tiles_h;
+  const int t = live ? item % (tiles_w * tiles_h) : 0, b = live ? item / (tiles_w * tiles_h) : 0;
+  const int h0 = (t / tiles_w) * kBTH, w0 = (t % tiles_w) * kBTW;
+  const int th = min(kBTH, H - h0), tw = min(kBTW, W - w0);
+  const int lane = pcnn::lane_id();
+  const int r0 = live ? lo[b] : 0, r1 = live ? hi[b] : -1;
+  auto bits_of = [&](int r, uint32_t (&rm)[kBTH], uint32_t (&cm)[kBTW], uint32_t& ror, uint32_t& cor) {
+    ror = cor = 0;
+#pragma unroll
+    for (int i = 0; i < kBTH; i++) rm[i] = 0;
+#pragma unroll
+    for (int j = 0; j < kBTW; j++) cm[j] = 0;
+    if (r > r1 || geo[(size_t)r * 8] != b) return (int)0;
+#pragma unroll
+    for (int i = 0; i < kBTH; i++)
+      if (i < th) ror |= rm[i] = rowbits[(size_t)r * H + h0 + i];
+#pragma unroll
+    for (int j = 0; j < kBTW; j++)
+      if (j < tw) cor |= cm[j] = colbits[(size_t)r * W + w0 + j];
+    return (int)__popc(ror) * (int)__popc(cor);
+  };
+  int total = 0;
+  for (int rb = r0; rb <= r1; rb += 64) {
+    uint32_t rm[kBTH], cm[kBTW], ror, cor;
+    total += bits_of(rb + lane, rm, cm, ror, cor);
+  }
+  total = pcnn::wave_sum(total);
+  if (lane == 0) s_total[wave] = total;
+  __syncthreads();
+  if (threadIdx.x == 0) {
+    int sum = 0;
+    for (int i = 0; i < kPlanWaves; i++) sum += s_total[i];
+    s_base = sum > 0 ? atomicAdd(cursor, sum) : 0;
+  }
+  __syncthreads();
+  int base = s_base;
+  for (int i = 0; i < wave; i++) base += s_total[i];
+  if (!live) return;
+  if (lane == 0) {
+    if (item == 0) cursor[1] = kBTH;
+    first[item] = total > 0 ? min(base, ent_cap) : 0;
+    count[item] = total > 0 ? max(min(total, ent_cap - base), 0) : 0;
+  }
+  if (total == 0) return;
+  for (int rb = r0; rb <= r1; rb += 64) {
+    const int r = rb + lane;
+    uint32_t rm[kBTH], cm[kBTW], ror, cor;
+    const int cnt = bits_of(r, rm, cm, ror, cor);
+    int off = cnt;
+#pragma unroll
+    for (int d = 1; d < 64; d <<= 1) {
+      const int v = __shfl_up(off, d, 64);
+      if (lane >= d) off += v;
+    }
+    const int round_total = __shfl(off, 63, 64);
+    int pos = base + off - cnt;
+    for (uint32_t rr = ror; rr; rr &= rr - 1) {
+      const int ph = __ffs(rr) - 1;
+      for (uint32_t cc = cor; cc; cc &= cc - 1) {
+        const int pw = __ffs(cc) - 1;
+        uint32_t cmask = 0, m = 0;
+#pragma unroll
+        for (int j = 0; j < kBTW; j++) cmask |= ((cm[j] >> pw) & 1u) << j;
+#pragma unroll
+        for (int i = 0; i < kBTH; i++)
+          if ((rm[i] >> ph) & 1u) m |= cmask << (i * kBTW);
+        if (pos < ent_cap) ent[pos] = roi_plan::pack_entry((uint32_t)((r * PH + ph) * PW + pw), m);
+        pos++;
+      }
+    }
+    base += round_total;
+  }
+}
+
+template <int kBTH, int kBTW, bool PX, int CPL>
+__global__ void __launch_bounds__(64) k_roi_bwd_ent(const float* __restrict__ top_diff,
+                                                     const void* __restrict__ argmax, int B, int H, int W, int C,
+                                                     const int32_t* __restrict__ hdr,
+                                                     const int32_t* __restrict__ first,
+                                                     const int32_t* __restrict__ count,
+                                                     const uint32_t* __restrict__ ent, float* __restrict__ bottom) {
   constexpr int kBPix = kBTH * kBTW;
-  __shared__ int2 ent[kBCap];
-  __shared__ int sh_total;
+  constexpr int kBBatch = 16 / CPL;
+  static_assert(64 % (2 * kBBatch) == 0, "a fetch pair never straddles a 64-entry block");
+  constexpr int kChunk = 64 * CPL;
+  constexpr int kAW = PX ? CPL / 2 : CPL;
+  static_assert(kBPix <= 8, "the entry's pixel mask is one byte");
   const int tiles_w = (W + kBTW - 1) / kBTW, tiles_h = (H + kBTH - 1) / kBTH;
-  const int nchunk = (C + kBChunk - 1) / kBChunk;
+  const int nchunk = (C + kChunk - 1) / kChunk;
   const int ipx = (int)((gridDim.x + 7) / 8);
   int id = (int)(blockIdx.x % 8) * ipx + (int)(blockIdx.x / 8);
   if (id >= B * tiles_w * tiles_h * nchunk) return;
@@ -280,138 +381,93 @@
   const int t = id % (tiles_w * tiles_h), b = id / (tiles_w * tiles_h);
   const int h0 = (t / tiles_w) * kBTH, w0 = (t % tiles_w) * kBTW;
   const int th = min(kBTH, H - h0), tw = min(kBTW, W - w0);
-  const int lane = pcnn::lane_id(), wave = threadIdx.x >> 6;
-  const int c = chunk * kBChunk + 2 * threadIdx.x;
+  const int lane = pcnn::lane_id();
+  const int c = chunk * kChunk + CPL * lane;
   const bool cok = c < C;
-  float2 acc[kBPix];
+  float acc[kBPix][CPL];
   int expv[kBPix];
 #pragma unroll
   for (int p = 0; p < kBPix; p++) {
-    acc[p] = make_float2(0.f, 0.f);
+#pragma unroll
+    for (int j = 0; j < CPL; j++) acc[p][j] = 0.f;
     const int pix = (h0 + p / kBTW) * W + w0 + p % kBTW;
     expv[p] = PX ? pix : pix * C + c;
   }
   constexpr int kNext = PX ? 0 : 1;
-  const int r0 = lo[b], r1 = hi[b];
   const __amdgpu_buffer_rsrc_t rs_t = __builtin_amdgcn_make_buffer_rsrc((void*)top_diff, (short)0, 0x7fffffff, 0x00020000);
   const __amdgpu_buffer_rsrc_t rs_a = __builtin_amdgcn_make_buffer_rsrc((void*)argmax, (short)0, 0x7fffffff, 0x00020000);
   const unsigned voff = cok ? (unsigned)c * 4u : 0x80000000u;
   const unsigned voff_a = cok ? (unsigned)c * (PX ? 2u : 4u) : 0x80000000u;
-  for (int rb = r0; rb <= r1; rb += 64) {
-    uint32_t rbits = 0;
-    uint32_t cbits = 0;
-    const int r = rb + lane;
-    if (wave == 0 && r <= r1) {
-      const int32_t* gg = geo + (size_t)r * 8;
-      RoiGeo g;
-      g.b = gg[0]; g.sw = gg[2]; g.sh = gg[3]; g.ew = gg[4]; g.eh = gg[5];
-      g.bin_h = __int_as_float(gg[6]);
-      g.bin_w = __int_as_float(gg[7]);
-      if (g.b == b && g.sh <= h0 + th - 1 && g.eh >= h0 && g.sw <= w0 + tw - 1 && g.ew >= w0) {
-        for (int i = 0; i < th; i++) {
-          const int h = h0 + i;
-          if (h < g.sh || h > g.eh) continue;
-          int s0 = (int)floorf((float)(h - g.sh) / g.bin_h), e0 = (int)ceilf((float)(h - g.sh + 1) / g.bin_h);
-          s0 = min(max(s0, 0), PH);
-          e0 = min(max(e0, 0), PH);
-          for (int ph = s0; ph < e0; ph++) rbits |= 1u << (ph * kBTH + i);
-        }
-        for (int j = 0; j < tw; j++) {
-          const int w = w0 + j;
-          if (w < g.sw || w > g.ew) continue;
-          int s0 = (int)floorf((float)(w - g.sw) / g.bin_w), e0 = (int)ceilf((float)(w - g.sw + 1) / g.bin_w);
-          s0 = min(max(s0, 0), PW);
-          e0 = min(max(e0, 0), PW);
-          for (int pw = s0; pw < e0; pw++) cbits |= 1u << (pw * kBTW + j);
+  struct Words { uint32_t w[kAW]; };
+  struct Vals { float v[CPL]; };
+  const int total = hdr[1] == kBTH ? count[id] : 0;
+  if (total > 0) {
+    const uint32_t* __restrict__ el = ent + first[id];
+    const int cbytes = C * 4;
+    uint32_t wA = el[min(lane, total - 1)];
+    uint32_t wB = total > 64 ? el[min(64 + lane, total - 1)] : 0u;
+    auto fetch = [&](int e0, uint32_t& my, Words (&av)[kBBatch], Vals (&dv)[kBBatch]) {
+      my = (e0 & 64) ? wB : wA;
+#pragma unroll
+      for (int k = 0; k < kBBatch; k++) {
+        const int so = (int)(__builtin_amdgcn_readlane(my, (e0 & 63) + k) >> 8) * cbytes;
+        const int so_a = PX ? so >> 1 : so;
+        if constexpr (kAW == 1)
+          av[k].w[0] = __builtin_amdgcn_raw_buffer_load_b32(rs_a, voff_a, so_a, 0);
+        else if constexpr (kAW == 2)
+          av[k] = __builtin_bit_cast(Words, __builtin_amdgcn_raw_buffer_load_b64(rs_a, voff_a, so_a, 0));
+        else
+          av[k] = __builtin_bit_cast(Words, __builtin_amdgcn_raw_buffer_load_b128(rs_a, voff_a, so_a, 0));
+        if constexpr (CPL == 2)
+          dv[k] = __builtin_bit_cast(Vals, __builtin_amdgcn_raw_buffer_load_b64(rs_t, voff, so, 0));
+        else
+          dv[k] = __builtin_bit_cast(Vals, __builtin_amdgcn_raw_buffer_load_b128(rs_t, voff, so, 0));
+      }
+    };
+    auto accumulate = [&](int e0, uint32_t my, const Words (&av)[kBBatch], const Vals (&dv)[kBBatch]) {
+#pragma unroll
+      for (int k = 0; k < kBBatch; k++) {
+        if (e0 + k >= total) break;
+        const uint32_t m = __builtin_amdgcn_readlane(my, (e0 & 63) + k) & 0xFFu;
+        int a[CPL];
+#pragma unroll
+        for (int j = 0; j < CPL; j++)
+          a[j] = PX ? (int)((av[k].w[j / 2] >> (16 * (j & 1))) & 0xFFFFu) : (int)av[k].w[PX ? 0 : j];
+#pragma unroll
+        for (int q = 0; q < kBPix; q++) {
+          if (!((m >> q) & 1)) continue;
+#pragma unroll
+          for (int j = 0; j < CPL; j++) acc[q][j] += a[j] == expv[q] + j * kNext ? dv[k].v[j] : 0.f;
         }
       }
-    }
-    const uint64_t hits = __ballot(rbits && cbits);
-    for (int g0 = 0; g0 < 64; g0 += kBGroup) {
-      if (wave == 0) {
-        const uint64_t gm = hits & (((1ull << kBGroup) - 1) << g0);
-        const bool mine = (gm >> lane) & 1;
-        int cnt = 0;
-        if (mine) {
-          int nph = 0, npw = 0;
-          for (int ph = 0; ph < PH; ph++) nph += ((rbits >> (ph * kBTH)) & ((1u << kBTH) - 1)) != 0;
-          for (int pw = 0; pw < PW; pw++) npw += ((cbits >> (pw * kBTW)) & ((1u << kBTW) - 1)) != 0;
-          cnt = nph * npw;
+    };
+    uint32_t myA, myB;
+    Words avA[kBBatch], avB[kBBatch];
+    Vals dvA[kBBatch], dvB[kBBatch];
+    fetch(0, myA, avA, dvA);
+    for (int e0 = 0; e0 < total; e0 += 2 * kBBatch) {
+      if (e0 + kBBatch < total) fetch(e0 + kBBatch, myB, avB, dvB);
+      accumulate(e0, myA, avA, dvA);
+      if (e0 + 2 * kBBatch < total) fetch(e0 + 2 * kBBatch, myA, avA, dvA);
+      if (e0 + kBBatch < total) accumulate(e0 + kBBatch, myB, avB, dvB);
+      const int nb = e0 + 2 * kBBatch + 64;
+      if (((e0 + 2 * kBBatch) & 63) == 0 && nb < total) {
+        const uint32_t v = el[min(nb + lane, total - 1)];
+        if (e0 & 64) wB = v; else wA = v;
+      }
+    }
+  }
+  if (cok) {
+#pragma unroll
+    for (int i = 0; i < kBTH; i++)
+#pragma unroll
+      for (int j = 0; j < kBTW; j++)
+        if (i < th && j < tw) {
+          float* o = bottom + (((size_t)b * H + h0 + i) * W + w0 + j) * C + c;
+          const float* v = acc[i * kBTW + j];
+          if (CPL == 2) *(float2*)o = make_float2(v[0], v[1]);
+          else *(float4*)o = make_float4(v[0], v[1], v[2], v[3]);
         }
-        int off = cnt;
-#pragma unroll
-        for (int d = 1; d < 64; d <<= 1) {
-          const int v = __shfl_up(off, d, 64);
-          if (lane >= d) off += v;
-        }
-        if (lane == 63) sh_total = off;
-        off -= cnt;
-        if (mine) {
-          const int rbase = r * PH;
-          for (int ph = 0; ph < PH; ph++) {
-            const uint32_t rm = (rbits >> (ph * kBTH)) & ((1u << kBTH) - 1);
-            if (!rm) continue;
-            for (int pw = 0; pw < PW; pw++) {
-              const uint32_t cm = (cbits >> (pw * kBTW)) & ((1u << kBTW) - 1);
-              if (!cm) continue;
-              uint32_t m = 0;
-#pragma unroll
-              for (int i = 0; i < kBTH; i++)
-                if ((rm >> i) & 1) m |= cm << (i * kBTW);
-              ent[off++] = make_int2(((rbase + ph) * PW + pw) * C, (int)m);
-            }
-          }
-        }
-      }
-      __syncthreads();
-      const int total = sh_total;
-      auto fetch = [&](int e0, int2& my, int2 (&av)[kBBatch], float2 (&dv)[kBBatch]) {
-        my = ent[min(e0 + (lane & (kBBatch - 1)), total - 1)];
-#pragma unroll
-        for (int k = 0; k < kBBatch; k++) {
-          const int so = __builtin_amdgcn_readlane(my.x, k) * 4;
-          if (PX) {
-            const unsigned a2 = __builtin_amdgcn_raw_buffer_load_b32(rs_a, voff_a, so >> 1, 0);
-            av[k] = make_int2((int)(a2 & 0xFFFFu), (int)(a2 >> 16));
-          } else {
-            av[k] = __builtin_bit_cast(int2, __builtin_amdgcn_raw_buffer_load_b64(rs_a, voff_a, so, 0));
-          }
-          dv[k] = __builtin_bit_cast(float2, __builtin_amdgcn_raw_buffer_load_b64(rs_t, voff, so, 0));
-        }
-      };
-      auto accumulate = [&](int e0, const int2& my, const int2 (&av)[kBBatch], const float2 (&dv)[kBBatch]) {
-#pragma unroll
-        for (int k = 0; k < kBBatch; k++) {
-          if (e0 + k >= total) break;
-          const uint32_t m = (uint32_t)__builtin_amdgcn_readlane(my.y, k);
-#pragma unroll
-          for (int q = 0; q < kBPix; q++) {
-            if (!((m >> q) & 1)) continue;
-            acc[q].x += av[k].x == expv[q] ? dv[k].x : 0.f;
-            acc[q].y += av[k].y == expv[q] + kNext ? dv[k].y : 0.f;
-          }
-        }
-      };
-      if (total > 0) {
-        int2 myA, myB, avA[kBBatch], avB[kBBatch];
-        float2 dvA[kBBatch], dvB[kBBatch];
-        fetch(0, myA, avA, dvA);
-        for (int e0 = 0; e0 < total; e0 += 2 * kBBatch) {
-          if (e0 + kBBatch < total) fetch(e0 + kBBatch, myB, avB, dvB);
-          accumulate(e0, myA, avA, dvA);
-          if (e0 + 2 * kBBatch < total) fetch(e0 + 2 * kBBatch, myA, avA, dvA);
-          if (e0 + kBBatch < total) accumulate(e0 + kBBatch, myB, avB, dvB);
-        }
-      }
-      __syncthreads();
-    }
-  }
-  if (cok) {
-#pragma unroll
-    for (int i = 0; i < kBTH; i++)
-#pragma unroll
-      for (int j = 0; j < kBTW; j++)
-        if (i < th && j < tw) *(float2*)(bottom + (((size_t)b * H + h0 + i) * W + w0 + j) * C + c) = acc[i * kBTW + j];
   }
 }
 
@@ -554,6 +610,130 @@
          pcnn::align_up((size_t)(R_cap > 0 ? R_cap : 1) * 8 * sizeof(int32_t), 256) + 256;
 }
 
+extern "C" size_t pcnn_roi_pool_bwd_plan_size(int B, int H, int W, int C, int R_cap, int pooled_h, int pooled_w,
+                                              int tile_h) {
+  if (!roi_plan::plannable(B, H, W, C, R_cap, pooled_h, pooled_w) || tile_h < 0 || tile_h > 2) return 0;
+  return roi_plan::layout(B, H, W, R_cap, pooled_h, pooled_w, roi_plan::tile_h(B, H, W, C, tile_h)).bytes;
+}
+
+extern "C" size_t pcnn_roi_pool_bwd_plan_entry_cap(int B, int H, int W, int C, int R_cap, int pooled_h, int pooled_w,
+                                                   int tile_h) {
+  if (!roi_plan::plannable(B, H, W, C, R_cap, pooled_h, pooled_w) || tile_h < 0 || tile_h > 2) return 0;
+  return roi_plan::entry_cap(H, W, R_cap, pooled_h, pooled_w, roi_plan::tile_h(B, H, W, C, tile_h));
+}
+
+namespace {
+struct PlanView {
+  int th;
+  int32_t *cursor, *lo, *hi, *geo, *first, *count;
+  uint8_t *rowbits, *colbits;
+  uint32_t* ent;
+  int ent_cap;
+};
+PlanView plan_view(void* plan, int B, int H, int W, int C, int R_cap, int PH, int PW, int tile_h) {
+  PlanView v;
+  v.th = roi_plan::tile_h(B, H, W, C, tile_h);
+  const roi_plan::Layout L = roi_plan::layout(B, H, W, R_cap, PH, PW, v.th);
+  char* p = (char*)plan;
+  v.cursor = (int32_t*)(p + L.cursor);
+  v.lo = (int32_t*)(p + L.lo);
+  v.hi = (int32_t*)(p + L.hi);
+  v.geo = (int32_t*)(p + L.geo);
+  v.rowbits = (uint8_t*)(p + L.rowbits);
+  v.colbits = (uint8_t*)(p + L.colbits);
+  v.first = (int32_t*)(p + L.first);
+  v.count = (int32_t*)(p + L.count);
+  v.ent = (uint32_t*)(p + L.ent);
+  v.ent_cap = (int)L.ent_cap;
+  return v;
+}
+}
+
+static int roi_pool_bwd_plan(const float* rois, int R_cap, int roi_stride, int batch_base,
+                             const int32_t* num_rois_dev, int B, int H, int W, int C, float spatial_scale, int pooled_h,
+                             int pooled_w, int tile_h, void* plan, size_t plan_bytes, hipStream_t st) {
+  PCNN_REQUIRE(rois && plan && roi_stride >= 5 && tile_h >= 0 && tile_h <= 2);
+  PCNN_REQUIRE(roi_plan::plannable(B, H, W, C, R_cap, pooled_h, pooled_w));
+  PCNN_REQUIRE(((uintptr_t)plan & 255) == 0);
+  const PlanView v = plan_view(plan, B, H, W, C, R_cap, pooled_h, pooled_w, tile_h);
+  PCNN_REQUIRE((size_t)v.ent_cap < (1ul << 30));
+  if (plan_bytes < roi_plan::layout(B, H, W, R_cap, pooled_h, pooled_w, v.th).bytes) return PCNN_ECAPACITY;
+  hipLaunchKernelGGL(k_roi_prep, dim3(1), dim3(1024), 0, st, rois, R_cap, roi_stride, batch_base, num_rois_dev, B,
+                     spatial_scale, pooled_h, pooled_w, v.geo, v.lo, v.hi, v.cursor);
+  if (R_cap > 0)
+    hipLaunchKernelGGL(k_roi_plan_bits, dim3(R_cap), dim3(128), 0, st, v.geo, R_cap, num_rois_dev, H, W, pooled_h,
+                       pooled_w, v.rowbits, v.colbits);
+  const long items = (long)B * roi_plan::tiles_of(H, W, v.th);
+  const unsigned nwg = (unsigned)((items + kPlanWaves - 1) / kPlanWaves);
+  if (v.th == 1)
+    hipLaunchKernelGGL(k_roi_plan_list<1>, dim3(nwg), dim3(64 * kPlanWaves), 0, st, v.geo, v.lo, v.hi, v.rowbits,
+                       v.colbits, B, H, W, pooled_h, pooled_w, v.cursor, v.first, v.count, v.ent, v.ent_cap);
+  else
+    hipLaunchKernelGGL(k_roi_plan_list<2>, dim3(nwg), dim3(64 * kPlanWaves), 0, st, v.geo, v.lo, v.hi, v.rowbits,
+                       v.colbits, B, H, W, pooled_h, pooled_w, v.cursor, v.first, v.count, v.ent, v.ent_cap);
+  PCNN_CHECK_LAUNCH();
+  return PCNN_OK;
+}
+
+extern "C" int pcnn_roi_pool_bwd_plan(const float* rois, int R_cap, int roi_stride, int batch_base,
+                                      const int32_t* num_rois_dev, int B, int H, int W, int C, float spatial_scale,
+                                      int pooled_h, int pooled_w, int tile_h, void* plan, size_t plan_bytes,
+                                      void* stream) {
+  return roi_pool_bwd_plan(rois, R_cap, roi_stride, batch_base, num_rois_dev, B, H, W, C, spatial_scale, pooled_h,
+                           pooled_w, tile_h, plan, plan_bytes, (hipStream_t)stream);
+}
+
+static bool roi_bwd_aligned(const float* top_diff, const void* argmax, bool px, const float* bottom_diff) {
+  return (((uintptr_t)top_diff | (uintptr_t)bottom_diff) & 7) == 0 && ((uintptr_t)argmax & (px ? 3 : 7)) == 0;
+}
+
+static int roi_pool_bwd_planned(const float* top_diff, const void* argmax, bool px, int B, int H, int W, int C,
+                                int R_cap, int pooled_h, int pooled_w, int tile_h, int lane_channels, const void* plan,
+                                size_t plan_bytes, float* bottom_diff, hipStream_t st) {
+  PCNN_REQUIRE(top_diff && argmax && plan && bottom_diff && tile_h >= 0 && tile_h <= 2);
+  PCNN_REQUIRE(roi_plan::plannable(B, H, W, C, R_cap, pooled_h, pooled_w));
+  PCNN_REQUIRE(roi_bwd_aligned(top_diff, argmax, px, bottom_diff) && ((uintptr_t)plan & 255) == 0);
+  PCNN_REQUIRE(!px || (long)H * W < 0xFFFF);
+  const PlanView v = plan_view((void*)plan, B, H, W, C, R_cap, pooled_h, pooled_w, tile_h);
+  if (plan_bytes < roi_plan::layout(B, H, W, R_cap, pooled_h, pooled_w, v.th).bytes) return PCNN_ECAPACITY;
+  const bool can4 = C % 4 == 0 && (((uintptr_t)top_diff | (uintptr_t)bottom_diff) & 15) == 0 &&
+                    ((uintptr_t)argmax & (px ? 7 : 15)) == 0;
+  PCNN_REQUIRE(lane_channels == 0 || lane_channels == 2 || (lane_channels == 4 && can4));
+  const bool wide = lane_channels == 4 || (lane_channels == 0 && can4 && roi_plan::wide_by_size(B, H, W, C, v.th));
+  const int nchunk = (C + (wide ? 256 : 128) - 1) / (wide ? 256 : 128);
+  const long items = (long)B * roi_plan::tiles_of(H, W, v.th) * nchunk;
+  const unsigned nwg = (unsigned)((items + 7) / 8 * 8);
+#define PCNN_RBW(TH, PXV, CPLV)                                                                                  \
+  pcnn::launch_last(k_roi_bwd_ent<TH, roi_plan::kTileW, PXV, CPLV>, dim3(nwg), dim3(64), 0, st, top_diff, argmax, B, \
+                    H, W, C, (const int32_t*)v.cursor, (const int32_t*)v.first, (const int32_t*)v.count,          \
+                    (const uint32_t*)v.ent, bottom_diff)
+#define PCNN_RBW2(TH, PXV) do { if (wide) PCNN_RBW(TH, PXV, 4); else PCNN_RBW(TH, PXV, 2); } while (0)
+  if (v.th == 1) {
+    if (px) PCNN_RBW2(1, true); else PCNN_RBW2(1, false);
+  } else {
+    if (px) PCNN_RBW2(2, true); else PCNN_RBW2(2, false);
+  }
+#undef PCNN_RBW2
+#undef PCNN_RBW
+  PCNN_CHECK_LAUNCH();
+  return PCNN_OK;
+}
+
+extern "C" int pcnn_roi_pool_bwd_planned(const float* top_diff, const int32_t* argmax, int B, int H, int W, int C,
+                                         int R_cap, int pooled_h, int pooled_w, int tile_h, int lane_channels,
+                                         const void* plan, size_t plan_bytes, float* bottom_diff, void* stream) {
+  return roi_pool_bwd_planned(top_diff, argmax, false, B, H, W, C, R_cap, pooled_h, pooled_w, tile_h, lane_channels, plan,
+                              plan_bytes, bottom_diff, (hipStream_t)stream);
+}
+
+extern "C" int pcnn_roi_pool_bwd_planned_px(const float* top_diff, const uint16_t* argmax_px, int B, int H, int W,
+                                            int C, int R_cap, int pooled_h, int pooled_w, int tile_h,
+                                            int lane_channels, const void* plan, size_t plan_bytes,
+                                            float* bottom_diff, void* stream) {
+  return roi_pool_bwd_planned(top_diff, argmax_px, true, B, H, W, C, R_cap, pooled_h, pooled_w, tile_h, lane_channels, plan,
+                              plan_bytes, bottom_diff, (hipStream_t)stream);
+}
+
 static int roi_pool_bwd(const float* top_diff, const void* argmax, bool px, int B, int H, int W, int C, int layout,
                         const float* rois, int R_cap, int roi_stride, int batch_base, const int32_t* num_rois_dev,
                         float spatial_scale, int pooled_h, int pooled_w, int pool_channel, float* bottom_diff,
@@ -562,44 +742,29 @@
   PCNN_REQUIRE(pooled_h > 0 && pooled_w > 0 && (layout == 0 || layout == 1) && R_cap >= 0);
   PCNN_REQUIRE(roi_stride >= 6 || (roi_stride == 5 && !pool_channel));
   PCNN_REQUIRE((long)H * W * C < (1l << 31));
+  hipStream_t st = (hipStream_t)stream;
+  const bool vec = layout == 0 && !pool_channel && roi_plan::plannable(B, H, W, C, R_cap, pooled_h, pooled_w) &&
+                   roi_bwd_aligned(top_diff, argmax, px, bottom_diff) && ((uintptr_t)workspace & 255) == 0;
+  PCNN_REQUIRE(!px || (vec && (long)H * W < 0xFFFF));
+  if (vec) {
+    const int rc = roi_pool_bwd_plan(rois, R_cap, roi_stride, batch_base, num_rois_dev, B, H, W, C, spatial_scale,
+                                     pooled_h, pooled_w, 0, workspace, workspace_bytes, st);
+    if (rc != PCNN_OK) return rc;
+    return roi_pool_bwd_planned(top_diff, argmax, px, B, H, W, C, R_cap, pooled_h, pooled_w, 0, 0, workspace,
+                                workspace_bytes, bottom_diff, st);
+  }
   if (workspace_bytes < pcnn_roi_pool_bwd_workspace_size(B, R_cap)) return PCNN_ECAPACITY;
-  hipStream_t st = (hipStream_t)stream;
   pcnn::Carve cv(workspace);
   int32_t* lo = cv.take<int32_t>(B);
   int32_t* hi = cv.take<int32_t>(B);
   int32_t* geo = cv.take<int32_t>((size_t)(R_cap > 0 ? R_cap : 1) * 8);
   hipLaunchKernelGGL(k_roi_prep, dim3(1), dim3(1024), 0, st, rois, R_cap, roi_stride, batch_base, num_rois_dev,
-                     B, spatial_scale, pooled_h, pooled_w, geo, lo, hi);
-  const int nchunk = (C + kBChunk - 1) / kBChunk;
-  const long wg24 = (long)B * ((H + 1) / 2) * ((W + 3) / 4) * nchunk;
-  const bool narrow = wg24 < PCNN_RBW_NARROW;
-#ifndef PCNN_RBW_TH
-#define PCNN_RBW_TH 2
-#endif
-  const int tbh = narrow ? 1 : PCNN_RBW_TH, tbw = 4;
-  const bool vec = layout == 0 && !pool_channel && C % 2 == 0 && pooled_h * tbh <= 32 && pooled_w * tbw <= 32 &&
-                   (long)H * W * C < (1l << 30) && (long)R_cap * pooled_h * pooled_w * C < (1l << 29) &&
-                   (((uintptr_t)top_diff | (uintptr_t)bottom_diff) & 7) == 0 && ((uintptr_t)argmax & (px ? 3 : 7)) == 0;
-  PCNN_REQUIRE(!px || (vec && (long)H * W < 0xFFFF));
-  if (vec) {
-    const int tiles = ((H + tbh - 1) / tbh) * ((W + tbw - 1) / tbw);
-    const unsigned nwg = (unsigned)((B * tiles * nchunk + 7) / 8 * 8);
-#define PCNN_RBW(TH, PXV)                                                                                  \
-  pcnn::launch_last(k_roi_bwd_ent<TH, 4, PXV>, dim3(nwg), dim3(64 * kBWaves), 0, st, top_diff, argmax, B, H, W, C, \
-                    geo, lo, hi, pooled_h, pooled_w, bottom_diff)
-    if (narrow) {
-      if (px) PCNN_RBW(1, true); else PCNN_RBW(1, false);
-    } else {
-      if (px) PCNN_RBW(PCNN_RBW_TH, true); else PCNN_RBW(PCNN_RBW_TH, false);
-    }
-#undef PCNN_RBW
-  } else {
-    if (hipMemsetAsync(bottom_diff, 0, (size_t)B * H * W * C * sizeof(float), st) != hipSuccess) return PCNN_EHIP;
-    const long npix = (long)B * H * W;
-    const int blocks = (int)((npix + 255) / 256 < 8192 ? (npix + 255) / 256 : 8192);
-    hipLaunchKernelGGL(k_roi_bwd_generic, dim3(blocks), dim3(256), 0, st, top_diff, (const int32_t*)argmax, B, H, W,
-                       C, layout, geo, pooled_h, pooled_w, pool_channel, lo, hi, bottom_diff);
-  }
+                     B, spatial_scale, pooled_h, pooled_w, geo, lo, hi, (int32_t*)nullptr);
+  if (hipMemsetAsync(bottom_diff, 0, (size_t)B * H * W * C * sizeof(float), st) != hipSuccess) return PCNN_EHIP;
+  const long npix = (long)B * H * W;
+  const int blocks = (int)((npix + 255) / 256 < 8192 ? (npix + 255) / 256 : 8192);
+  hipLaunchKernelGGL(k_roi_bwd_generic, dim3(blocks), dim3(256), 0, st, top_diff, (const int32_t*)argmax, B, H, W,
+                     C, layout, geo, pooled_h, pooled_w, pool_channel, lo, hi, bottom_diff);
   PCNN_CHECK_LAUNCH();
   return PCNN_OK;
 }
diff --git a/posecnn_amd/pipeline.py b/posecnn_amd/pipeline.py
--- a/posecnn_amd/pipeline.py
+++ b/posecnn_amd/pipeline.py
@@ -41,6 +41,12 @@
         px = pixel_argmax and max(self.h4 * self.w4, self.h5 * self.w5) < 0xFFFF
         adt = dict(dtype=torch.int16 if px else torch.int32, device=device)
 
+        lib = _lib.load()
+        shape5, shape4 = (B, self.h5, self.w5, channels), (B, self.h4, self.w4, channels)
+        plan_bytes = [lib.pcnn_roi_pool_bwd_plan_size(*s_, CAP, 7, 7, 0) for s_ in (shape5, shape4)]
+        if backward and not all(plan_bytes):
+            raise ValueError("PoseStep: the conv4 / conv5 shapes have no planned RoI-pool backward")
+
         def minibatch_set():
             return dict(hough=dict(box=torch.zeros((CAP, 7), **f32), pose=torch.zeros((CAP, 7), **f32),
                                    target=torch.zeros((CAP, D), **f32), weight=torch.zeros((CAP, D), **f32),
@@ -48,6 +54,8 @@
                         pool=torch.zeros((CAP, 7, 7, channels), **f32),
                         arg5=torch.zeros((CAP, 7, 7, channels), **adt),
                         arg4=torch.zeros((CAP, 7, 7, channels), **adt),
+                        plan5=torch.zeros((plan_bytes[0],), dtype=torch.uint8, device=device) if backward else None,
+                        plan4=torch.zeros((plan_bytes[1],), dtype=torch.uint8, device=device) if backward else None,
                         add_ws=None, prepped=False)
         self.fuse_loss_tail = fuse_loss_tail
         self.pipeline = bool(pipeline)
@@ -183,6 +191,7 @@
     def vote(self, label, vertex, extents, meta, gt, s=None):
         s = self._cur if s is None else s
         self._sets[s]["pooled"] = False
+        self._sets[s]["planned"] = False
         with self._t("hough_voting_gpu"):
             return hv.hough_voting_gpu_capacity(label, vertex, extents, meta, gt, self.is_train, self.vthr,
                                                 self.vper, self.skip, global_batch=self.global_batch,
@@ -208,11 +217,31 @@
     def pool_fwd(self, conv4, conv5, s=None):
         s = self._cur if s is None else s
         st = self._sets[s]
+        h = st["hough"]
         with self._t("roi_pool_fwd"):
-            rp.roi_pool_pair(conv5, 1.0 / 16.0, conv4, 1.0 / 8.0, st["hough"]["box"], 7, 7,
-                             num_rois=st["hough"]["num_rois"][1:2], out=(st["pool"], st["arg5"], st["arg4"]),
+            rp.roi_pool_pair(conv5, 1.0 / 16.0, conv4, 1.0 / 8.0, h["box"], 7, 7,
+                             num_rois=h["num_rois"][1:2], out=(st["pool"], st["arg5"], st["arg4"]),
                              batch_base=self.batch_base)
         st["pooled"] = True
+        if self.backward and not st.get("planned"):
+            self.plan_bwd(conv4, conv5, s=s)
+
+    def plan_bwd(self, conv4, conv5, s=None, side=False):
+        s = self._cur if s is None else s
+        st = self._sets[s]
+        h = st["hough"]
+        side_st = self.side_stream if side and self.timer is None and self.side_prep else None
+        if side_st is not None:
+            side_st.wait_stream(torch.cuda.current_stream())
+        with torch.cuda.stream(side_st or torch.cuda.current_stream()):
+            with self._t("roi_pool_plan"):
+                for plan, data, scale in ((st["plan5"], conv5, 1.0 / 16.0), (st["plan4"], conv4, 1.0 / 8.0)):
+                    rp.roi_pool_plan(h["box"], tuple(data.shape), 7, 7, scale, num_rois=h["num_rois"][1:2], out=plan,
+                                     batch_base=self.batch_base)
+            if side_st is not None:
+                st["plan_ev"] = st.get("plan_ev") or torch.cuda.Event()
+                st["plan_ev"].record(side_st)
+        st["planned"] = "side" if side_st is not None else "stream"
 
     def _front(self, inputs, s, stream=None):
         ctx = torch.cuda.stream(stream) if stream is not None else _nullctx()
@@ -445,10 +474,11 @@
         self._issue_pending_pool()
         dxp = self.dx.view(CAP, 7, 7, self.Ch)
         with self._t("roi_pool_bwd"):
-            rp.roi_pool_grad(conv5, h["box"], self.arg5, dxp, 7, 7, 1.0 / 16.0, 0, num_rois=nr, out=self.dconv5,
-                             batch_base=self.batch_base)
-            rp.roi_pool_grad(conv4, h["box"], self.arg4, dxp, 7, 7, 1.0 / 8.0, 0, num_rois=nr, out=self.dconv4,
-                             batch_base=self.batch_base)
+            st = self._sets[self._cur]
+            if st.get("planned") == "side":
+                main.wait_event(st["plan_ev"])
+            rp.roi_pool_grad_planned(st["plan5"], tuple(conv5.shape), CAP, self.arg5, dxp, 7, 7, out=self.dconv5)
+            rp.roi_pool_grad_planned(st["plan4"], tuple(conv4.shape), CAP, self.arg4, dxp, 7, 7, out=self.dconv4)
         if self._bump_drop_step:
             self.drop_step.add_(1)
             self._bump_drop_step = False
@@ -477,6 +507,8 @@
         self.draw_drop_masks()
         if self.side_prep:
             self.add_prep(inputs["points"], inputs["symmetry"])
+            if self.backward:
+                self.plan_bwd(inputs["conv4"], inputs["conv5"], side=True)
         return self._train(inputs)
 
     def _step_pipelined(self, inputs, next_inputs):
diff --git a/posecnn_amd/roi_pooling_layer/roi_pooling_op.py b/posecnn_amd/roi_pooling_layer/roi_pooling_op.py
--- a/posecnn_amd/roi_pooling_layer/roi_pooling_op.py
+++ b/posecnn_amd/roi_pooling_layer/roi_pooling_op.py
@@ -74,7 +74,10 @@
         B, C, H, W = bottom_data.shape
     R, stride = rois.shape
     lib = _lib.load()
-    ws = _lib.workspace(lib.pcnn_roi_pool_bwd_workspace_size(B, R), bottom_data.device, "roi_bwd")
+    need = max(lib.pcnn_roi_pool_bwd_workspace_size(B, R),
+               0 if layout != 0 or pool_channel else
+               lib.pcnn_roi_pool_bwd_plan_size(B, H, W, C, R, int(pooled_height), int(pooled_width), 0))
+    ws = _lib.workspace(need, bottom_data.device, "roi_bwd")
     dd = out if out is not None else torch.empty(bottom_data.shape, dtype=torch.float32, device=bottom_data.device)
     if argmax.dtype == torch.int16:
         if layout != 0 or pool_channel:
@@ -92,6 +95,38 @@
     return dd
 
 
+def roi_pool_plan(bottom_rois, data_shape, pooled_height, pooled_width, spatial_scale, num_rois=None, out=None,
+                  batch_base=0, tile_h=0):
+    _lib.require_gpu(bottom_rois)
+    rois = bottom_rois.contiguous().float()
+    B, H, W, C = data_shape
+    R, stride = rois.shape
+    lib = _lib.load()
+    need = lib.pcnn_roi_pool_bwd_plan_size(B, H, W, C, R, int(pooled_height), int(pooled_width), int(tile_h))
+    if need == 0:
+        raise ValueError("roi_pool_plan: this shape has no planned backward")
+    plan = out if out is not None else torch.empty(need, dtype=torch.uint8, device=rois.device)
+    rc = lib.pcnn_roi_pool_bwd_plan(_lib.ptr(rois), R, stride, int(batch_base), _lib.ptr(num_rois), B, H, W, C,
+                                    float(spatial_scale), int(pooled_height), int(pooled_width), int(tile_h),
+                                    _lib.ptr(plan), plan.numel(), _lib.stream_ptr())
+    _lib.check(rc, "roi_pool_plan")
+    return plan
+
+
+def roi_pool_grad_planned(plan, data_shape, num_rows, argmax, grad, pooled_height, pooled_width, out=None, tile_h=0,
+                          lane_channels=0):
+    _lib.require_gpu(plan, argmax, grad)
+    B, H, W, C = data_shape
+    lib = _lib.load()
+    dd = out if out is not None else torch.empty(tuple(data_shape), dtype=torch.float32, device=grad.device)
+    fn = lib.pcnn_roi_pool_bwd_planned_px if argmax.dtype == torch.int16 else lib.pcnn_roi_pool_bwd_planned
+    rc = fn(_lib.ptr(grad.contiguous()), _lib.ptr(argmax.contiguous()), B, H, W, C, int(num_rows),
+            int(pooled_height), int(pooled_width), int(tile_h), int(lane_channels), _lib.ptr(plan), plan.numel(),
+            _lib.ptr(dd), _lib.stream_ptr())
+    _lib.check(rc, "roi_pool_grad_planned")
+    return dd
+
+
 class RoiPoolFunction(torch.autograd.Function):
 
     @staticmethod
```

Result: no change. 4633 (median of 3 runs) (+0.1%).
